# marbl/Mash

Hardware: AMD Instinct MI355X
Metric: pairwise Mash distances/sec (s=1000) (higher is better)
Workload: dtype u64; 1 GPU; mash triangle all-vs-all, 100000 clustered synthetic sketches, k=21 s=1000, 4999950000 pairs/step, per-table job (index build + discover + fill + merge each step), row-block sharded x1; parallelism=rowblock1, rccl_ranks=0

## Files before the change

mash_amd/csrc/compare_dense.hip:

```cpp
#ifdef MG_HIP_EMU
#include "hipemu.h"
#else
#include <hip/hip_runtime.h>
#define MG_DYN_SHARED(T, name)                                   \
    extern __shared__ __align__(16) unsigned char name##_raw[]; \
    T *name = reinterpret_cast<T *>(name##_raw)
#endif
#include <stdint.h>

#include <cstdlib>

#ifndef MG_HIP_EMU
#include <rocprim/device/device_radix_sort.hpp>
#include <rocprim/device/device_select.hpp>
#include <rocprim/iterator/counting_iterator.hpp>
#endif

#include "compare_internal.h"

namespace mg {

#ifndef MG_HIP_EMU
__global__ __launch_bounds__(256) void dn_neighbor_kernel(const uint64_t *hashes, uint64_t stride, const uint32_t *cnt, uint32_t n,
                                                          uint8_t *link)
// ... 79 lines not shown
    if (lane == 63u) s_w[wid] = incl;
    __syncthreads();
    uint32_t base = 0;
    for (uint32_t k = 0; k < wid; k++) base += s_w[k];
    off[t] = base + incl - c;
    if (t == DN_SUBLISTS - 1u) total[0] = base + incl;
    atomicMax(&total[1], want);
}

__global__ __launch_bounds__(256) void dn_sublists_copy_kernel(const unsigned long long *key, const uint32_t *val, const uint32_t *cnt,
                                                               const uint32_t *off, uint32_t cap_sub, unsigned long long *key_out,
                                                               uint32_t *val_out)
{
    const uint32_t sub = blockIdx.x;
    const uint32_t c = cnt[sub] < cap_sub ? cnt[sub] : cap_sub, o = off[sub];
    for (uint32_t k = threadIdx.x; k < c; k += 256u) {
        key_out[o + k] = key[(uint64_t)sub * cap_sub + k];
        val_out[o + k] = val[(uint64_t)sub * cap_sub + k];
    }
}

__global__ __launch_bounds__(256) void dn_universe_split_kernel(const unsigned long long *key_sorted, uint32_t m, uint32_t *ulist,
                                                                uint32_t *ustart, uint32_t *uend)
{
    const uint32_t i = blockIdx.x * 256u + threadIdx.x;
    if (i >= m) return;
    const unsigned long long k = key_sorted[i];
    const uint32_t g = (uint32_t)(k >> 32);
    ulist[i] = (uint32_t)k;
    if (i == 0 || (uint32_t)(key_sorted[i - 1] >> 32) != g) ustart[g] = i;
    if (i + 1u == m || (uint32_t)(key_sorted[i + 1] >> 32) != g) uend[g] = i + 1u;
}

size_t dense_universe_temp_bytes(uint32_t cap)
{
    size_t b = 0;
    rocprim::radix_sort_pairs(nullptr, b, (const unsigned long long *)nullptr, (unsigned long long *)nullptr, (const uint32_t *)nullptr,
                              (uint32_t *)nullptr, (size_t)cap, 0u, 64u, (hipStream_t) nullptr);
    return b;
}

uint32_t dense_sublists() { return DN_SUBLISTS; }

hipError_t dense_find_leaders(const uint32_t *sorted_rows, const uint32_t *gs_of, const uint32_t *gend, const uint32_t *grp_of,
                              const DenseGroup *groups, uint32_t E, unsigned long long *key, uint32_t *val, uint32_t cap_sub,
                              unsigned long long *key_out, uint32_t *val_out, uint32_t *cnt, uint32_t *off, uint32_t *total,
                              hipStream_t stream)
{
    if (E == 0) return hipSuccess;
    hipError_t e = hipMemsetAsync(cnt, 0, DN_SUBLISTS * 4, stream);
    if (e == hipSuccess) e = hipMemsetAsync(total, 0, 8, stream);
    if (e != hipSuccess) return e;
    hipLaunchKernelGGL(dn_leaders_kernel, dim3((E + 255u) / 256u), dim3(256), 0, stream, sorted_rows, gs_of, gend, grp_of, groups, E, key, val, cap_sub,
                       cnt);
    e = hipGetLastError();
    if (e != hipSuccess) return e;
    return dense_join_leaders(key, val, cap_sub, key_out, val_out, cnt, off, total, stream);
}

hipError_t dense_join_leaders(const unsigned long long *key, const uint32_t *val, uint32_t cap_sub, unsigned long long *key_out, uint32_t *val_out,
                              const uint32_t *cnt, uint32_t *off, uint32_t *total, hipStream_t stream)
{
    hipLaunchKernelGGL(dn_sublists_scan_kernel, dim3(1), dim3(DN_SUBLISTS), 0, stream, cnt, cap_sub, off, total);
    hipLaunchKernelGGL(dn_sublists_copy_kernel, dim3(DN_SUBLISTS), dim3(256), 0, stream, key, val, cnt, (const uint32_t *)off, cap_sub, key_out, val_out);
    return hipGetLastError();
}

hipError_t dense_sort_universes(const unsigned long long *key, const uint32_t *val, uint32_t m, void *temp, size_t temp_bytes,
                                unsigned long long *key_sorted, uint32_t *ulist, uint32_t *upos, uint32_t *ustart, uint32_t *uend,
                                uint32_t group_bits, hipStream_t stream)
{
    if (m == 0) return hipSuccess;
    hipError_t e = rocprim::radix_sort_pairs(temp, temp_bytes, key, key_sorted, val, upos, (size_t)m, 0u, 32u + group_bits, stream);
    if (e != hipSuccess) return e;
    hipLaunchKernelGGL(dn_universe_split_kernel, dim3((m + 255u) / 256u), dim3(256), 0, stream, (const unsigned long long *)key_sorted, m, ulist,
                       ustart, uend);
    return hipGetLastError();
}

#endif

constexpr uint32_t DN_CX_MASK = 0x7FFFu, DN_CX_FLAG = 0x8000u;

template <uint32_t DN_EK>
__global__ __launch_bounds__(256) void dn_encode_kernel(const uint32_t *off, const uint32_t *code_img, uint32_t *pos_img, uint32_t rs,
                                                        const uint32_t *grp_of, const DenseGroup *groups, const uint32_t *ulist,
                                                        const uint32_t *upos, unsigned long long *gdata, uint32_t wstride, uint16_t *ext,
                                                        uint32_t xs, uint32_t n, uint32_t ul_in_lds)
{
    MG_DYN_SHARED(uint32_t, lds);
    const uint32_t bid = blockIdx.x;
    const uint32_t row = (bid & ~63u) | ((bid & 7u) << 3) | ((bid >> 3) & 7u);
    const uint32_t tid = threadIdx.x, lane = tid & 63u, wid = tid >> 6;
    if (row >= n) return;
    const uint32_t g = grp_of[row];
    if (g == 0xFFFFFFFFu) return;
    const DenseGroup G = groups[g];
    const uint32_t W = G.W, u = G.u;
    uint32_t *mask32 = lds, *hist = lds + 2u * W, *gap8 = hist + W + 1u, *ovf = gap8 + 16u * W, *pl32 = ovf + W, *scr = pl32 + 8u * W;
    uint32_t *ull = lds + 28u * wstride + 9u;
    for (uint32_t i = tid; i < 28u * W + 1u; i += 256u) lds[i] = 0;
    const uint32_t *ulg = ulist + G.ustart, *up = upos + G.ustart;
    if (ul_in_lds)
        for (uint32_t i = tid; i < u; i += 256u) ull[i] = ulg[i];
    const uint32_t *ul = ul_in_lds ? ull : ulg;
    __syncthreads();
    const uint32_t cnt = off[row + 1] - off[row];
    uint16_t *xrow = ext + (uint64_t)(G.xrow0 + (row - G.g0)) * xs;
    uint32_t nx = 0;
    if constexpr (DN_EK == 1) {
        for (uint32_t base = 0; base < cnt; base += 256u) {
            const uint32_t p = base + tid;
            uint32_t idx = 0;
            bool extra = false;
            if (p < cnt) {
                const uint64_t img = (uint64_t)row * rs + p;
                const uint32_t gs = code_img[img] >> 1;
                uint32_t lo = 0, hi = u;
                while (lo < hi) {
                    const uint32_t mid = (lo + hi) >> 1;
                    if (ul[mid] < gs) lo = mid + 1; else hi = mid;
                }
                idx = lo;
                if (lo < u && ul[lo] == gs) {
                    atomicOr(&mask32[idx >> 5], 1u << (idx & 31u));
                    pos_img[img] = up[idx];
                } else {
                    extra = true;
                }
            }
            const uint64_t bal = __ballot(extra);
            const uint32_t before = (uint32_t)__popcll(bal & ((1ull << lane) - 1ull));
            if (lane == 0) scr[wid] = (uint32_t)__popcll(bal);
            __syncthreads();
            uint32_t woff = 0;
            for (uint32_t k = 0; k < wid; k++) woff += scr[k];
            const uint32_t total = scr[0] + scr[1] + scr[2] + scr[3];
            if (extra) {
                xrow[nx + woff + before] = (uint16_t)idx;
                atomicAdd(&hist[idx >> 6], 1u);
                atomicAdd(&gap8[idx >> 2], 1u << (8u * (idx & 3u)));
            }
            nx += total;
            __syncthreads();
        }
    } else {
        for (uint32_t base = 0; base < cnt; base += 256u * DN_EK) {
            const uint32_t p0 = base + tid * DN_EK;
            const uint32_t nv = p0 < cnt ? (cnt - p0 < DN_EK ? cnt - p0 : DN_EK) : 0u;
            uint32_t xidx[DN_EK];
            uint32_t nxt = 0;
            if (nv) {
                const uint64_t img0 = (uint64_t)row * rs + p0;
                const uint4 c0 = *reinterpret_cast<const uint4 *>(code_img + img0), c1 = *reinterpret_cast<const uint4 *>(code_img + img0 + 4u);
                const uint32_t code[DN_EK] = {c0.x, c0.y, c0.z, c0.w, c1.x, c1.y, c1.z, c1.w};
                uint4 *pp = reinterpret_cast<uint4 *>(pos_img + img0);
                const uint4 q0 = pp[0], q1 = pp[1];
                uint32_t pv[DN_EK] = {q0.x, q0.y, q0.z, q0.w, q1.x, q1.y, q1.z, q1.w};
                uint32_t pos = 0;
                {
                    const uint32_t gs0 = code[0] >> 1;
                    uint32_t lo = 0, hi = u;
                    while (lo < hi) {
                        const uint32_t mid = (lo + hi) >> 1;
                        if (ul[mid] < gs0) lo = mid + 1; else hi = mid;
                    }
                    pos = lo;
                }
    #pragma unroll
                for (uint32_t e = 0; e < DN_EK; e++) {
                    if (e < nv) {
                        const uint32_t gs = code[e] >> 1;
                        {
                            uint32_t lo = pos, hi = pos, step = 1;
                            while (hi < u && ul[hi] < gs) {
                                lo = hi + 1u;
                                hi += step;
                                step <<= 1;
                            }
                            hi = hi < u ? hi : u;
                            while (lo < hi) {
                                const uint32_t mid = (lo + hi) >> 1;
                                if (ul[mid] < gs) lo = mid + 1u; else hi = mid;
                            }
                            pos = lo;
                        }
                        if (pos < u && ul[pos] == gs) {
                            atomicOr(&mask32[pos >> 5], 1u << (pos & 31u));
                            pv[e] = up[pos];
                        } else {
    #pragma unroll
                            for (uint32_t j = 0; j < DN_EK; j++)
                                if (j == nxt) xidx[j] = pos;
                            nxt++;
                        }
                    }
                }
                pp[0] = make_uint4(pv[0], pv[1], pv[2], pv[3]);
                pp[1] = make_uint4(pv[4], pv[5], pv[6], pv[7]);
            }
            uint32_t incl = nxt;
    #pragma unroll
            for (uint32_t d = 1; d < 64u; d <<= 1) {
                const uint32_t y = __shfl_up(incl, d);
                if (lane >= d) incl += y;
            }
            if (lane == 63u) scr[wid] = incl;
            __syncthreads();
            uint32_t woff = 0;
            for (uint32_t k = 0; k < wid; k++) woff += scr[k];
            const uint32_t total = scr[0] + scr[1] + scr[2] + scr[3];
            const uint32_t at0 = nx + woff + incl - nxt;
    #pragma unroll
            for (uint32_t j = 0; j < DN_EK; j++) {
                if (j < nxt) {
                    const uint32_t idx = xidx[j];
                    xrow[at0 + j] = (uint16_t)idx;
                    atomicAdd(&hist[idx >> 6], 1u);
                    atomicAdd(&gap8[idx >> 2], 1u << (8u * (idx & 3u)));
                }
            }
            nx += total;
            __syncthreads();
        }
    }
    __syncthreads();
    const uint32_t jb = (row - G.g0) >> 7, bl = (row - G.g0) & 127u;
    const uint64_t bw = dense_block_words(W);
    unsigned long long *blk = gdata + G.data_off + (uint64_t)jb * bw;
    uint16_t *cxp = reinterpret_cast<uint16_t *>(blk + 128ull * W), *totp = cxp + (W + 1u) * 128u;
    unsigned long long *xpl = blk + dense_block_planes(W);
    for (uint32_t i = tid; i < 16u * W; i += 256u) {
        const uint32_t four = gap8[i], w = i >> 4, q = i & 15u;
        uint32_t bits[4] = {0u, 0u, 0u, 0u}, over = 0;
#pragma unroll
        for (uint32_t e = 0; e < 4u; e++) {
            const uint32_t c = (four >> (8u * e)) & 255u;
            over |= c >= 16u ? 1u : 0u;
#pragma unroll
            for (uint32_t j = 0; j < 4u; j++) bits[j] |= ((c >> j) & 1u) << ((4u * q + e) & 31u);
        }
        if (over || (q == 0 && hist[w] >= 256u)) ovf[w] = 1u;
#pragma unroll
        for (uint32_t j = 0; j < 4u; j++)
            if (bits[j]) atomicOr(&pl32[2u * (4u * w + j) + (q >> 3)], bits[j]);
    }
    __syncthreads();
    for (uint32_t i = tid; i < 4u * W; i += 256u) xpl[i * 128u + bl] = (unsigned long long)pl32[2u * i] | ((unsigned long long)pl32[2u * i + 1u] << 32);
    if (tid == 0) {
        uint32_t run = 0, all = 0;
        for (uint32_t w = 0; w <= W; w++) {
            cxp[w * 128u + bl] = (uint16_t)(run | ((w > 0 && ovf[w - 1u]) ? DN_CX_FLAG : 0u));
            totp[w * 128u + bl] = (uint16_t)all;
            if (w < W) {
                run += hist[w];
                all += hist[w] + (uint32_t)__popc(mask32[2u * w]) + (uint32_t)__popc(mask32[2u * w + 1u]);
            }
        }
    }
    for (uint32_t w = tid; w < W; w += 256u)
        blk[w * 128u + bl] = (unsigned long long)mask32[2u * w] | ((unsigned long long)mask32[2u * w + 1u] << 32);
}

hipError_t launch_dense_encode(const uint32_t *off, const uint32_t *code_img, uint32_t *pos_img, uint32_t rs, const uint32_t *grp_of,
                               const DenseGroup *groups, const uint32_t *ulist, const uint32_t *upos, unsigned long long *gdata,
                               uint16_t *ext, uint32_t xs, uint32_t n, uint32_t wmax, hipStream_t stream, int ul_mode)
{
    if (n == 0) return hipSuccess;
    const size_t fixed = ((size_t)28 * wmax + 9) * 4, with_ul = fixed + (size_t)wmax * 64 * 4;
    const bool ul_in_lds = ul_mode == 0 ? false : ul_mode == 1 ? with_ul <= 150 * 1024 : with_ul <= 40 * 1024;
    const size_t smem = ul_in_lds ? with_ul : fixed;
    auto go = [&](auto kern) -> hipError_t {
        hipError_t e = hipFuncSetAttribute(reinterpret_cast<const void *>(kern), hipFuncAttributeMaxDynamicSharedMemorySize, (int)smem);
        if (e != hipSuccess) return e;
        hipLaunchKernelGGL(kern, dim3((n + 63u) & ~63u), dim3(256), smem, stream, off, code_img, pos_img, rs, grp_of, groups, ulist, upos, gdata, wmax, ext, xs,
                           n, ul_in_lds ? 1u : 0u);
        return hipGetLastError();
    };
    return rs >= 4096u ? go(dn_encode_kernel<8>) : go(dn_encode_kernel<1>);
}



__device__ __forceinline__ uint32_t dn_count_add(uint32_t x, uint32_t acc)
{
#ifdef MG_HIP_EMU
    return (uint32_t)__popc(x) + acc;
#else
    uint32_t d;
    asm("v_bcnt_u32_b32 %0, %1, %2" : "=v"(d) : "v"(x), "v"(acc));
    return d;
#endif
}

__device__ __forceinline__ uint32_t dn_low_bits(uint32_t x, uint32_t y)
{
#ifdef MG_HIP_EMU
    return x & ((1u << y) - 1u);
#else
    return __builtin_amdgcn_ubfe(x, 0u, y);
#endif
}

template <uint32_t NP>
__device__ __forceinline__ uint32_t dn_descend(uint32_t base, uint32_t s, uint32_t u1, uint32_t A0, uint32_t B0, uint32_t A1, uint32_t B1,
                                               uint32_t A2, uint32_t B2, uint32_t A3, uint32_t B3)
{
    uint32_t pos = 0;
#pragma unroll
    for (uint32_t bit = 16u; bit != 0u; bit >>= 1) {
        const uint32_t y = pos + bit;
        uint32_t c = dn_count_add(dn_low_bits(B0, y), dn_count_add(dn_low_bits(A0, y), dn_count_add(dn_low_bits(u1, y), base)));
        if (NP >= 1u) c += 2u * dn_count_add(dn_low_bits(B1, y), (uint32_t)__popc(dn_low_bits(A1, y)));
        if (NP >= 3u)
            c += 4u * dn_count_add(dn_low_bits(B2, y), (uint32_t)__popc(dn_low_bits(A2, y))) +
                 8u * dn_count_add(dn_low_bits(B3, y), (uint32_t)__popc(dn_low_bits(A3, y)));
        pos = c < s ? y : pos;
    }
    return pos;
}

__device__ __forceinline__ uint32_t dn_resolve(unsigned long long un, unsigned long long mab, uint32_t fprev, uint32_t s, uint32_t w, bool lists,
                                               const unsigned long long *xpa, const unsigned long long *xpb, const uint16_t *xa,
                                               const uint16_t *xb, uint32_t ca0, uint32_t na, uint32_t cb0, uint32_t nb)
{
    if (__ballot(lists) == 0) {
        const unsigned long long a0 = xpa[512u * w], a1 = xpa[512u * w + 128u], a2 = xpa[512u * w + 256u], a3 = xpa[512u * w + 384u];
        const unsigned long long b0 = xpb[512u * w], b1 = xpb[512u * w + 128u], b2 = xpb[512u * w + 256u], b3 = xpb[512u * w + 384u];
        const bool p1 = __ballot((a1 | b1) != 0ull) != 0, p23 = __ballot((a2 | a3 | b2 | b3) != 0ull) != 0;
        const uint32_t ulo = (uint32_t)un, uhi = (uint32_t)(un >> 32);
        uint32_t c31 = dn_count_add((uint32_t)b0, dn_count_add((uint32_t)a0, dn_count_add(ulo & 0x7FFFFFFFu, fprev)));
        if (p1 || p23) c31 += 2u * dn_count_add((uint32_t)b1, (uint32_t)__popc((uint32_t)a1));
        if (p23)
            c31 += 4u * dn_count_add((uint32_t)b2, (uint32_t)__popc((uint32_t)a2)) + 8u * dn_count_add((uint32_t)b3, (uint32_t)__popc((uint32_t)a3));
        const bool upper = c31 < s;
        const uint32_t base = upper ? c31 + (ulo >> 31) : fprev;
        const uint32_t u1 = (upper ? uhi : ulo) << 1;
        const uint32_t A0 = upper ? (uint32_t)(a0 >> 32) : (uint32_t)a0, B0 = upper ? (uint32_t)(b0 >> 32) : (uint32_t)b0;
        uint32_t pos;
        if (!p1 && !p23) {
            pos = dn_descend<0>(base, s, u1, A0, B0, 0, 0, 0, 0, 0, 0);
        } else {
            const uint32_t A1 = upper ? (uint32_t)(a1 >> 32) : (uint32_t)a1, B1 = upper ? (uint32_t)(b1 >> 32) : (uint32_t)b1;
            if (!p23) {
                pos = dn_descend<1>(base, s, u1, A0, B0, A1, B1, 0, 0, 0, 0);
            } else {
                const uint32_t A2 = upper ? (uint32_t)(a2 >> 32) : (uint32_t)a2, B2 = upper ? (uint32_t)(b2 >> 32) : (uint32_t)b2;
                const uint32_t A3 = upper ? (uint32_t)(a3 >> 32) : (uint32_t)a3, B3 = upper ? (uint32_t)(b3 >> 32) : (uint32_t)b3;
                pos = dn_descend<3>(base, s, u1, A0, B0, A1, B1, A2, B2, A3, B3);
            }
        }
        const uint32_t mlo = (uint32_t)mab, mhi = (uint32_t)(mab >> 32);
        return upper ? dn_count_add(dn_low_bits(mhi, pos), (uint32_t)__popc(mlo)) : (uint32_t)__popc(dn_low_bits(mlo, pos));
    }
    uint32_t lo = 0, hi = 63;
    const uint32_t wbase = w << 6;
    while (lo < hi) {
        const uint32_t mid = (lo + hi) >> 1;
        uint32_t c = fprev + (uint32_t)__popcll(un & ((1ull << mid) - 1ull));
// ... 292 lines not shown
```

mash_amd/csrc/compare_internal.h:

```cpp
#pragma once
#ifdef MG_HIP_EMU
#include "hipemu.h"
#else
#include <hip/hip_runtime.h>
#endif
#include <stdint.h>

namespace mg {

struct MergedTile {
    uint32_t rows[32];
    uint32_t col0, col1;
};

struct CompareArgs {
    const uint64_t *row_hashes;
    const uint32_t *row_nhash;
    const uint64_t *col_hashes;
    const uint32_t *col_nhash;
    const uint32_t *row_pfx;
    const uint32_t *col_pfx;
    const MergedTile *mtiles;
    uint2 *out;
    uint64_t row_stride, col_stride;
    uint64_t row_pfx_stride, col_pfx_stride;
    uint64_t row_begin, row_end;
    uint64_t ncols;
    uint64_t out_base;
    uint32_t s;
    uint32_t rows_per_tile;
    uint32_t triangle;
    uint32_t unroll;
    uint32_t pfx_shr;
    uint32_t nbuckets;
    unsigned long long *dbg;
    const uint32_t *row_win;
    const uint32_t *col_win;
    uint32_t win, nwin;
    uint32_t win_lo, win_hi;
    uint32_t win_ecap;
    uint8_t *win_mask;
    uint32_t win_kmax;
    uint32_t xcd_remap;
    uint32_t stage_pack;
};

bool compare_merged_supported(uint32_t s);
uint32_t compare_merged_rows(uint32_t s);
hipError_t launch_compare_merged(const CompareArgs &a, uint32_t ntiles, hipStream_t stream);
uint32_t compare_window_rows(uint32_t s);
uint32_t compare_window_entries();
uint32_t compare_window_row_entries();
hipError_t launch_window_offsets(const uint32_t *pfx, uint64_t pfx_stride, const uint32_t *nhash, uint64_t n, uint32_t s,
                                 uint32_t nwin, uint32_t delta, uint32_t *out, hipStream_t stream);
hipError_t launch_table_max(const uint64_t *hashes, const uint32_t *nhash, uint64_t n, uint64_t stride,
                            unsigned long long *out_max, hipStream_t stream);
hipError_t launch_row_classes(const uint64_t *hashes, const uint32_t *nhash, uint64_t n, uint64_t stride,
                              uint8_t *out, unsigned long long *last_out, hipStream_t stream);
uint64_t compare_pfx_stride(uint64_t s);
hipError_t launch_make_prefix(const uint64_t *hashes, const uint32_t *nhash, uint64_t n, uint64_t s,
                              uint64_t pfx_stride, uint32_t shr, uint32_t *out, hipStream_t stream);
hipError_t launch_compare_generic(const CompareArgs &a, hipStream_t stream);

struct DenseGroup;
struct SparseArgs {
    const uint32_t *sorted_rows;
    const uint32_t *lo_img;
    const uint32_t *hi_img;
    uint32_t lo_shift;
    const uint32_t *off;
    const uint32_t *row_img;
    const uint32_t *col_img;
    const uint32_t *col_cnt_off;
    uint32_t rs_row, rs_col;
    uint32_t row_begin, row_end;
    uint32_t ncols;
    uint32_t triangle;
    uint32_t s;
    uint64_t out_base;
    uint2 *cand;
    uint64_t cand_cap;
    unsigned long long *counters;
    uint2 *out;
    uint2 *res;
    unsigned long long *seg_base;
    uint32_t *seg_cnt;
    uint32_t *chunk_inc;
    const uint32_t *rep;
    const uint32_t *cls_of;
    const uint32_t *cls_off;
    const uint32_t *cls_rows;
    const uint32_t *gend;
    const uint32_t *order;
    const uint32_t *inv;
    const uint32_t *dn_grp_of;
    const DenseGroup *dn_groups;
};
size_t sparse_dup_temp_bytes(uint32_t n);
hipError_t launch_sparse_dup_suspects(const unsigned long long *dig, const uint32_t *cnt, uint32_t n, void *temp, size_t temp_bytes,
                                      unsigned long long *dig_sorted, uint32_t *rows_sorted, uint32_t *flags, uint32_t *nflag,
                                      hipStream_t stream);
size_t sparse_order_temp_bytes(uint32_t n);
hipError_t launch_sparse_row_order(const uint32_t *off, const uint32_t *code_img, const uint32_t *gend, const uint32_t *rep, uint32_t n,
                                   uint32_t rs, void *temp, size_t temp_bytes, unsigned long long *key_a, unsigned long long *key_b,
                                   uint32_t *order, hipStream_t stream);
size_t sparse_order_slice_temp_bytes(uint32_t n);
hipError_t launch_sparse_order_slice(const uint32_t *order, uint32_t n, uint32_t rb, uint32_t re, void *temp, size_t temp_bytes,
                                     uint32_t *out, uint32_t *count_out, hipStream_t stream);
hipError_t launch_sparse_class_pairs(uint2 *out, const uint32_t *cls_rows, const uint32_t *cls_first, const uint32_t *off,
                                     const uint32_t *rep, uint32_t members, uint32_t row_begin, uint32_t row_end, uint64_t out_base,
                                     const uint32_t *inv, hipStream_t stream);
hipError_t launch_sparse_row_digest(const uint64_t *hashes, uint64_t stride, const uint32_t *cnt, uint32_t n,
                                    unsigned long long *digest, hipStream_t stream);
hipError_t launch_sparse_row_gate(const uint64_t *hashes, uint64_t stride, const uint32_t *cnt, uint32_t n, unsigned long long *digest,
                                  hipStream_t stream);
hipError_t launch_sparse_row_equal(const uint64_t *hashes, uint64_t stride, const uint32_t *cnt, const uint2 *pairs, uint32_t npairs,
                                   uint32_t *equal, hipStream_t stream);
hipError_t launch_sparse_row_counts(const uint32_t *nhash, uint32_t n, uint32_t cap, uint32_t *cnt, hipStream_t stream);
size_t sparse_offsets_temp_bytes(uint32_t n);
hipError_t launch_sparse_offsets(const uint32_t *cnt, const uint32_t *inv, uint32_t n, void *temp, uint32_t *off, hipStream_t stream);
size_t sparse_sort_temp_bytes(uint32_t E, uint32_t end_bit, uint32_t begin_bit);
uint32_t sparse_img_stride(uint32_t s);
hipError_t sparse_build_index(const uint64_t *hashes, uint64_t stride, const uint32_t *off, uint32_t n, uint32_t E,
                              uint32_t rs, uint32_t end_bit, void *temp, size_t temp_bytes, uint64_t *keys_a,
                              uint32_t *idx_a, uint64_t *keys_sorted, uint32_t *idx_sorted, uint32_t *head, uint32_t *gs_of,
                              uint32_t *sorted_rows, uint32_t *gend, uint32_t *code_img, uint32_t *pos_img, void *stat_scratch,
                              uint32_t begin_bit, void *tie_scratch, unsigned long long *incidences, uint32_t *max_group, uint32_t *groups,
                              uint32_t *bad, uint32_t *tie_overflow, hipStream_t stream, const uint32_t *rowmap = nullptr);
size_t sparse_stat_scratch_bytes();
uint32_t sparse_sort_begin_bit(uint32_t E, uint32_t end_bit, const char *forced_bits, bool all_bits);
size_t sparse_tie_scratch_bytes();
hipError_t launch_sparse_locate(const uint64_t *qhashes, uint64_t qstride, const uint32_t *qoff, uint32_t q_begin, uint32_t nq,
                                const uint64_t *keys_sorted, const uint32_t *gend, uint32_t E, uint32_t rs, uint32_t *qlo_img,
                                uint32_t *qhi_img, uint32_t *qcode_img, hipStream_t stream);
bool sparse_discover_supported(uint32_t ncols_max);
hipError_t launch_sparse_discover(const SparseArgs &a, bool count_only, hipStream_t stream);
hipError_t launch_sparse_merge(const SparseArgs &a, uint64_t expect, uint32_t cus, hipStream_t stream);
bool sparse_merge_rows_supported(uint32_t rs_row);
size_t sparse_scan_temp_bytes(uint32_t nrows);
hipError_t launch_sparse_merge_rows(const SparseArgs &a, uint64_t expect, uint32_t *chunks, void *temp, size_t temp_bytes,
                                    hipStream_t stream, bool *windowed_out = nullptr);
hipError_t launch_sparse_scatter(const SparseArgs &a, uint64_t expect, uint32_t cus, hipStream_t stream);
size_t sparse_gather_temp_bytes(uint32_t nrows);
hipError_t launch_sparse_gather_rows(const SparseArgs &a, uint32_t *cnt_by_row, uint32_t *row_base, void *temp, size_t temp_bytes, uint32_t row_add,
                                     uint2 *rc_out, uint2 *counts_out, hipStream_t stream);
size_t sparse_edges_temp_bytes(uint64_t K);
uint64_t sparse_edges_blocks(uint64_t K);
hipError_t launch_sparse_list_edges(const uint2 *rc, const uint2 *counts, uint64_t K, uint32_t *blk_cnt, uint32_t *blk_off, void *temp, size_t temp_bytes,
                                    uint4 *edges, unsigned long long *total, hipStream_t stream);
uint64_t sparse_fill_chunks(uint64_t pairs);
constexpr uint32_t kFillStop = 0x80000000u;
hipError_t launch_sparse_fill_chunks(uint2 *out, uint64_t pairs, uint32_t numer, uint32_t denom, uint32_t blocks, uint32_t naps, uint32_t *ctr,
                                     hipStream_t stream, uint32_t threads = 256);
hipError_t launch_sparse_fill_value(uint2 *out, uint64_t pairs, uint32_t numer, uint32_t denom, uint32_t blocks_per_cu, uint32_t cus,
                                    hipStream_t stream);
hipError_t launch_sparse_merge_pack(const SparseArgs &a, uint64_t expect, uint32_t *chunks, void *temp, size_t temp_bytes, bool *used,
                                    hipStream_t stream, uint32_t *pack_min_out = nullptr);
hipError_t launch_sparse_fill_short(uint2 *out, const uint32_t *short_rows, const uint32_t *short_rcnt, uint32_t nshort_rows,
                                    const uint32_t *short_cols, const uint32_t *short_ccnt, uint32_t nshort_cols,
                                    uint32_t row_begin, uint32_t ncols, uint32_t triangle, uint64_t out_base, uint32_t s,
                                    const uint32_t *inv, hipStream_t stream);

struct DenseGroup {
    uint32_t g0, g1;
    uint32_t ustart, u;
    uint32_t W;
    uint32_t xrow0;
    uint64_t data_off;
};
struct DenseTile { uint32_t group, row0, cblk; };
#ifdef __HIPCC__
__host__ __device__
#endif
static inline uint64_t dense_block_planes(uint32_t W) { return 128ull * W + 64ull * (W + 1u); }
#ifdef __HIPCC__
__host__ __device__
#endif
static inline uint64_t dense_block_words(uint32_t W) { return dense_block_planes(W) + 512ull * W; }
struct DenseList {
    const uint32_t *row_base = nullptr, *row_cnt = nullptr;
    uint2 *rc = nullptr, *counts = nullptr;
    uint32_t row_first = 0;
};
hipError_t launch_dense_neighbors(const uint64_t *hashes, uint64_t stride, const uint32_t *cnt, uint32_t n, uint8_t *link,
                                  hipStream_t stream);
size_t dense_universe_temp_bytes(uint32_t cap);
uint32_t dense_sublists();
hipError_t dense_find_leaders(const uint32_t *sorted_rows, const uint32_t *gs_of, const uint32_t *gend, const uint32_t *grp_of,
                              const DenseGroup *groups, uint32_t E, unsigned long long *key, uint32_t *val, uint32_t cap_sub,
                              unsigned long long *key_out, uint32_t *val_out, uint32_t *cnt, uint32_t *off, uint32_t *total,
                              hipStream_t stream);
hipError_t dense_join_leaders(const unsigned long long *key, const uint32_t *val, uint32_t cap_sub, unsigned long long *key_out, uint32_t *val_out,
                              const uint32_t *cnt, uint32_t *off, uint32_t *total, hipStream_t stream);
hipError_t dense_sort_universes(const unsigned long long *key, const uint32_t *val, uint32_t m, void *temp, size_t temp_bytes,
                                unsigned long long *key_sorted, uint32_t *ulist, uint32_t *upos, uint32_t *ustart, uint32_t *uend,
                                uint32_t group_bits, hipStream_t stream);
hipError_t launch_dense_encode(const uint32_t *off, const uint32_t *code_img, uint32_t *pos_img, uint32_t rs, const uint32_t *grp_of,
                               const DenseGroup *groups, const uint32_t *ulist, const uint32_t *upos, unsigned long long *gdata,
                               uint16_t *ext, uint32_t xs, uint32_t n, uint32_t wmax, hipStream_t stream, int ul_mode = -1);
size_t dense_pairs_lds(uint32_t W, uint32_t rows);
uint32_t dense_rows_per_tile(uint64_t wave_rows);
uint32_t dense_max_words();
hipError_t launch_dense_pairs(const DenseTile *tiles, uint32_t ntiles, uint32_t rows_per_tile, const DenseGroup *groups,
                              const unsigned long long *gdata, bool use_lists, const uint16_t *ext, uint32_t xs,
                              uint32_t s, uint32_t wmax, uint32_t row_begin, uint32_t row_end, uint64_t out_base, const uint32_t *inv, uint2 *out,
                              hipStream_t stream, const DenseList *list = nullptr);
size_t dense_cluster_temp_bytes(uint32_t n);
hipError_t dense_cluster_rows(const uint64_t *hashes, uint64_t stride, const uint32_t *cnt, uint32_t n, void *temp, size_t temp_bytes,
                              unsigned long long *key_a, unsigned long long *key_b, uint32_t *row_a, uint32_t *row_b, uint32_t *lab_a,
                              uint32_t *lab_b, uint32_t *inv, uint32_t *label_sorted, hipStream_t stream, uint32_t split = 0);
hipError_t launch_dense_gather_rows(const uint64_t *hashes, uint64_t stride, const uint32_t *inv, uint32_t n, uint64_t *out, hipStream_t stream);
hipError_t launch_dense_group_rows(const DenseGroup *groups, uint32_t ng, uint32_t n, uint32_t *grp_of, uint32_t *lead_rows, hipStream_t stream);

struct JoinSide {
    const uint2 *grp = nullptr;
    const uint32_t *ent = nullptr;
    const uint32_t *goff = nullptr;
    const uint32_t *gend = nullptr;
    const uint32_t *thr = nullptr;
};
struct JoinArgs {
    JoinSide rows, cols;
    const uint32_t *row_cnt_off, *col_cnt_off;
    const uint32_t *rep, *col_rep;
    const uint32_t *inv;
    uint2 *out;
    uint64_t out_base;
    uint64_t ntiles;
    uint32_t ncols;
    uint32_t row_begin, row_end;
    uint32_t bi0;
    uint32_t ncb;
    uint32_t triangle, s;
    uint32_t tiles_per_wg = 1;
};
size_t join_order_temp_bytes(uint32_t nrows);
hipError_t join_order_rows(const uint32_t *img, uint32_t rs, const uint32_t *cnt_off, const uint32_t *rep, const uint32_t *inv, const uint32_t *gend,
                           const uint32_t *sorted_rows, uint32_t nrows, void *temp, size_t temp_bytes, uint32_t *lab, unsigned long long *key_a,
                           unsigned long long *key_b, uint32_t *val_a, uint32_t *perm, uint32_t *src, uint32_t *map, hipStream_t stream, uint32_t split = 0);
uint32_t join_block_rows();
uint32_t join_levels();
size_t join_build_temp_bytes(uint64_t slots);
hipError_t join_build_lists(const uint32_t *img, uint32_t rs, const uint32_t *cnt_off, const uint32_t *rep, uint32_t nrows, uint32_t s, uint32_t E,
                            bool only_shared, void *temp, size_t temp_bytes, unsigned long long *key_a, unsigned long long *key_b, uint32_t *val_a,
                            uint32_t *val_b, uint2 *grp, uint32_t *goff, uint32_t *gend, uint32_t *thr, const uint32_t **ent_out, hipStream_t stream);
hipError_t launch_join_levels(const uint32_t *img, uint32_t rs, const uint32_t *cnt_off, const uint32_t *rep, uint32_t nrows, uint32_t s,
                              uint32_t *thr, hipStream_t stream);
hipError_t launch_join_shared(const uint32_t *lo_img, const uint32_t *hi_img, uint32_t lo_shift, uint32_t rs, const uint32_t *cnt_off,
                              uint32_t row_begin, uint32_t row_end, unsigned long long *sum, hipStream_t stream);
hipError_t launch_join_tiles(const JoinArgs &a, hipStream_t stream);

struct FilterArgs {
    const uint2 *counts;
    const uint32_t *min_numer;
    uint32_t *seg_count;
    unsigned long long *seg_off;
    uint4 *edges;
    uint64_t pairs;
    uint64_t first_row;
    uint64_t ncols;
    uint64_t win_lo, win_n;
    uint32_t s;
    uint32_t triangle;
};
uint64_t filter_segments(uint64_t pairs);
hipError_t launch_filter_count(const FilterArgs &a, unsigned long long *total, hipStream_t stream);
hipError_t launch_filter_write(const FilterArgs &a, hipStream_t stream);

}
```

mash_amd/csrc/compare_sparse.hip:

```cpp
#include <stdint.h>

#include <cstdlib>
#include <cstring>

#include "compare_internal.h"
#ifdef MG_HIP_EMU
#include <numeric>
#define SP_DYN_U32(name, align) MG_DYN_SHARED(uint32_t, name)
#else
#include <hip/hip_runtime.h>
#include <rocprim/device/device_radix_sort.hpp>
#include <rocprim/device/device_scan.hpp>
#include <rocprim/device/device_select.hpp>
#include <rocprim/iterator/counting_iterator.hpp>
#define SP_DYN_U32(name, align) extern __shared__ align uint32_t name[]
#endif
#include "copy_gate.h"

namespace mg {

#ifndef MG_HIP_EMU


__global__ __launch_bounds__(256) void sp_fill_entries_kernel(const uint64_t *hashes, uint64_t stride, const uint32_t *rowmap, const uint32_t *off,
// ... 517 lines not shown
        e = hipGetLastError();
        if (e != hipSuccess) return e;
    }
    hipLaunchKernelGGL(sp_heads_kernel, dim3(blocks), dim3(256), 0, stream, keys_sorted, idx_sorted, E, head, bad);
    e = hipGetLastError();
    if (e != hipSuccess) return e;
    e = rocprim::inclusive_scan(temp, temp_bytes, (const uint32_t *)head, gs_of, (size_t)E, sp_max_u32(), stream);
    if (e != hipSuccess) return e;
    {
        const uint64_t total = (uint64_t)n * rs;
        uint64_t fb = (total + 1023) / 1024;
        if (fb > 8192) fb = 8192;
        hipLaunchKernelGGL(sp_fill_u32_kernel, dim3((uint32_t)fb), dim3(256), 0, stream, code_img, total, 0xFFFFFFFFu);
        e = hipGetLastError();
        if (e != hipSuccess) return e;
    }
    e = hipMemsetAsync(stat_scratch, 0, sparse_stat_scratch_bytes(), stream);
    if (e != hipSuccess) return e;
    hipLaunchKernelGGL(sp_index_scatter_kernel, dim3(blocks), dim3(256), 0, stream, (const uint32_t *)idx_sorted, (const uint32_t *)gs_of, E, rs,
                       sorted_rows, gend, code_img, pos_img, static_cast<SpStatSlot *>(stat_scratch));
    e = hipGetLastError();
    if (e != hipSuccess) return e;
    hipLaunchKernelGGL(sp_stat_reduce_kernel, dim3(1), dim3(256), 0, stream, static_cast<const SpStatSlot *>(stat_scratch), incidences, max_group,
                       groups);
    return hipGetLastError();
}

#endif


__global__ __launch_bounds__(256) void sp_locate_kernel(const uint64_t *qhashes, uint64_t qstride, const uint32_t *qoff,
                                                        uint32_t q_begin, uint32_t nq, const uint64_t *keys_sorted,
                                                        const uint32_t *gend, uint32_t E, uint32_t rs, uint32_t *qlo_img,
                                                        uint32_t *qhi_img, uint32_t *qcode_img)
{
    const uint32_t q = blockIdx.x;
    if (q >= nq) return;
    const uint32_t cnt = qoff[q + 1] - qoff[q];
    const uint64_t *src = qhashes + (uint64_t)(q_begin + q) * qstride;
    for (uint32_t p = threadIdx.x; p < cnt; p += 256) {
        const uint64_t v = src[p];
        uint32_t lo = 0, hi = E;
        while (lo < hi) {
            const uint32_t mid = lo + ((hi - lo) >> 1);
            if (keys_sorted[mid] < v) lo = mid + 1; else hi = mid;
        }
        const bool found = lo < E && keys_sorted[lo] == v;
        const uint64_t at = (uint64_t)q * rs + p;
        qcode_img[at] = found ? (lo << 1) + 1u : (lo << 1);
        qlo_img[at] = lo;
        qhi_img[at] = found ? gend[lo] : lo;
    }
}


__device__ __forceinline__ uint32_t sp_class_span(const SparseArgs &a, uint32_t c, uint32_t row, uint32_t &first)
{
    const uint32_t k = a.cls_of[c];
    if (k == 0xFFFFFFFFu) { first = 0xFFFFFFFFu; return 1u; }
    const uint32_t lo = a.cls_off[k], hi = a.cls_off[k + 1];
    first = lo;
    if (!a.triangle) return hi - lo;
    uint32_t l = lo, h = hi;
    while (l < h) {
        const uint32_t mid = (l + h) >> 1;
        if (a.cls_rows[mid] < row) l = mid + 1; else h = mid;
    }
    return l - lo;
}

template <bool COUNT_ONLY, bool DEDUP>
__global__ __launch_bounds__(256) void sp_discover_kernel(SparseArgs a)
{
    SP_DYN_U32(bm, );
    __shared__ uint32_t s_w[4];
    __shared__ unsigned long long s_base;
    __shared__ unsigned long long s_inc[4];
    const uint32_t row = a.order ? a.order[blockIdx.x] : a.row_end - 1u - blockIdx.x;
    const uint32_t tid = threadIdx.x, lane = tid & 63u, wid = tid >> 6;
    const uint32_t ncols = a.triangle ? row : a.ncols;
    const uint32_t W = (ncols + 31u) >> 5;
    const uint32_t er = (DEDUP && a.triangle) ? a.rep[row] : row;
    const bool copy = DEDUP && a.triangle && er != row;
    const uint32_t cnt = a.off[er + 1] - a.off[er];
    if (cnt == 0 || ncols == 0) return;
    if (!copy) {
        int any = 0;
        for (uint32_t p = tid; p < cnt; p += 256u) {
            const uint64_t at = (uint64_t)er * a.rs_row + p;
            any |= (a.lo_img[at] >> a.lo_shift) != a.hi_img[at];
        }
        if (__syncthreads_or(any) == 0) return;
    }
    for (uint32_t w = tid; w < W; w += 256) bm[w] = 0;
    __syncthreads();
    unsigned long long inc = 0;
    constexpr uint32_t SHORT = 6;
    for (uint32_t base = wid * 64u; base < cnt; base += 256u) {
        const uint32_t p = base + lane;
        uint2 lh = make_uint2(0u, 0u);
        if (p < cnt) {
            const uint64_t at = (uint64_t)er * a.rs_row + p;
            lh = make_uint2(a.lo_img[at] >> a.lo_shift, a.hi_img[at]);
            if (copy) lh.y = a.gend[lh.x];
        }
        const uint32_t len = lh.y - lh.x;
        inc += len;
        if (len != 0 && len <= SHORT) {
            for (uint32_t t = 0; t < len; t++) {
                const uint32_t r = a.sorted_rows[lh.x + t];
                if (copy && r >= row) break;
                if (copy && r == er) continue;
                if (!((bm[r >> 5] >> (r & 31u)) & 1u)) atomicOr(&bm[r >> 5], 1u << (r & 31u));
            }
        }
        auto mark = [&](uint32_t r) {
            if (copy && (r >= row || r == er)) return;
            if (!((bm[r >> 5] >> (r & 31u)) & 1u)) atomicOr(&bm[r >> 5], 1u << (r & 31u));
        };
        uint64_t longm = __ballot(len > SHORT);
        while (longm != 0) {
            uint32_t lo4[4], hi4[4], r4[4];
#pragma unroll
            for (int k = 0; k < 4; k++) {
                lo4[k] = hi4[k] = 0;
                if (longm != 0) {
                    const int l = __builtin_ctzll(longm);
                    longm &= longm - 1;
                    lo4[k] = (uint32_t)__builtin_amdgcn_readlane((int)lh.x, l);
                    hi4[k] = (uint32_t)__builtin_amdgcn_readlane((int)lh.y, l);
                }
                r4[k] = lo4[k] + lane < hi4[k] ? a.sorted_rows[lo4[k] + lane] : 0xFFFFFFFFu;
            }
#pragma unroll
            for (int k = 0; k < 4; k++) {
                if (r4[k] != 0xFFFFFFFFu) mark(r4[k]);
                for (uint32_t q = lo4[k] + 64u + lane; q < hi4[k]; q += 64u) mark(a.sorted_rows[q]);
            }
        }
    }
    __syncthreads();
    const uint32_t per = (W + 255u) / 256u;
    const uint32_t w0 = tid * per, w1 = w0 + per < W ? w0 + per : W;
    uint32_t mine = 0;
    for (uint32_t w = w0; w < w1; w++) {
        if (!DEDUP) {
            mine += (uint32_t)__popc(bm[w]);
        } else {
            uint32_t bits = bm[w];
            while (bits != 0) {
                const uint32_t c = (w << 5) + (uint32_t)__builtin_ctz(bits);
                bits &= bits - 1;
                uint32_t first;
                mine += sp_class_span(a, c, row, first);
            }
        }
    }
    uint32_t incl = mine;
#pragma unroll
    for (int d = 1; d < 64; d <<= 1) {
        const uint32_t t = __shfl_up(incl, d);
        if (lane >= (uint32_t)d) incl += t;
    }
    for (int d = 32; d > 0; d >>= 1) inc += __shfl_xor(inc, d);
    if (lane == 63) s_w[wid] = incl;
    if (lane == 0) s_inc[wid] = inc;
    __syncthreads();
    uint32_t woff = 0;
    for (uint32_t w = 0; w < wid; w++) woff += s_w[w];
// ... 885 lines not shown
```

mash_amd/csrc/host_compare.cpp:

```cpp
#include "cut_internal.h"
#include "index_build.h"
#ifdef IX_PHASE_CLOCKS
namespace mg { void index_dump_clocks(); }
#endif
#include "sort_bits.h"
#include "topk_internal.h"
#include "knn_internal.h"
#include <type_traits>


int table_max(mg_ctx *ctx, const mg_table *t, uint64_t *out)
{
    if (!t->have_max) {
        unsigned long long *d = nullptr;
        HIP_TRY(ctx, hipMalloc(&d, 8));
        hipError_t e = hipMemsetAsync(d, 0, 8, ctx->stream);
        if (e == hipSuccess) e = mg::launch_table_max(t->hashes, t->nhash, t->n, t->s, d, ctx->stream);
        unsigned long long h = 0;
        if (e == hipSuccess) e = hipMemcpyAsync(&h, d, 8, hipMemcpyDeviceToHost, ctx->stream);
        if (e == hipSuccess) e = hipStreamSynchronize(ctx->stream);
        hipFree(d);
        if (e != hipSuccess) return fail(ctx, MG_ERR_HIP, std::string("table max: ") + hipGetErrorString(e));
        t->maxval = h;
        t->have_max = true;
// ... 507 lines not shown
        }
    }
    aside_wgs = wgs; aside_naps = naps; aside_threads = threads;
    ctx->aside_all_copies = [this](uint32_t c) { aside_other_constant(c); };
    uint64_t late_from = 300000000ull;
    if (const char *e = ctx_opt(ctx, "MASHGPU_FILL_ASIDE_AT_SORT")) late_from = strtoull(e, nullptr, 10);
    if (cols->n * std::min<uint64_t>(cols->s, s) >= late_from) {
        ctx->aside_at_sort = [this]() { (void)aside_start(); };
        return MG_OK;
    }
    return aside_start();
}

int SparseJobRun::aside_start()
{
    ctx->aside_at_sort = nullptr;
    if (prefilled) return MG_OK;
    HIP_TRY(ctx, hipMemsetAsync(ctx->aux_ctr, 0, 128, ctx->stream));
    HIP_TRY(ctx, hipEventRecord(ctx->aux_go, ctx->stream));
    HIP_TRY(ctx, hipStreamWaitEvent(ctx->aux, ctx->aux_go, 0));
    const bool copies = triangle && aside_copies != 0;
    return aside_launch(copies ? aside_copies : 0u, copies ? aside_copies : s, ctx->aux_ctr);
}

int SparseJobRun::aside_launch(uint32_t numer, uint32_t denom, uint32_t *ctr)
{
    prof_begin(ctx, ctx->prof_fill_aside, ctx->aux);
    HIP_TRY(ctx, mg::launch_sparse_fill_chunks(reinterpret_cast<uint2 *>(out_dev), pairs, numer, denom, aside_wgs, aside_naps, ctr, ctx->aux, aside_threads));
    prof_end(ctx, ctx->prof_fill_aside, ctx->aux);
    HIP_TRY(ctx, hipEventRecord(ctx->aux_done, ctx->aux));
    aside_numer = numer; aside_denom = denom; aside_ctr = ctr;
    prefilled = true;
    return MG_OK;
}

void SparseJobRun::aside_other_constant(uint32_t c)
{
    aside_copies = c;
    if (!prefilled || !triangle) return;
    if (hipMemsetAsync(aside_ctr, 0x80, 4, ctx->stream) != hipSuccess || aside_launch(c, c, ctx->aux_ctr + 16) != MG_OK) (void)hipGetLastError();
}

int SparseJobRun::end_prefill(bool finish)
{
    ctx->aside_all_copies = nullptr;
    ctx->aside_at_sort = nullptr;
    if (!prefilled) return MG_OK;
    prefilled = false;
    hipError_t e;
    if (finish) e = mg::launch_sparse_fill_chunks(reinterpret_cast<uint2 *>(out_dev), pairs, aside_numer, aside_denom, (uint32_t)ctx->cu_count * 16u, 0u, aside_ctr, ctx->stream);
    else e = hipMemsetAsync(aside_ctr, 0x80, 4, ctx->stream);
    const hipError_t e2 = hipStreamWaitEvent(ctx->stream, ctx->aux_done, 0);
    if (e != hipSuccess || e2 != hipSuccess) return fail(ctx, MG_ERR_HIP, std::string("compare (fill beside the build): ") + hipGetErrorString(e != hipSuccess ? e : e2));
    return MG_OK;
}

int SparseJobRun::row_side()
{
    a.sorted_rows = ix->sorted_rows;
    a.col_img = ix->code_img;
    a.col_cnt_off = ix->off;
    a.rs_col = ix->rs;
    a.ncols = (uint32_t)cols->n;
    a.triangle = triangle ? 1u : 0u;
    a.s = s;
    a.out = reinterpret_cast<uint2 *>(out_dev);
    a.counters = ix->counters;
    a.rep = ix->rep;
    a.cls_of = ix->cls_of;
    a.cls_off = ix->cls_off;
    a.cls_rows = ix->cls_rows;
    a.gend = ix->gend;
    a.inv = ix->inv;
    a.dn_grp_of = (job && triangle && !ix->dgroups_host.empty()) ? ix->grp_of : nullptr;
    a.dn_groups = a.dn_grp_of ? ix->dgroups : nullptr;
    a.res = nullptr;
    a.seg_base = nullptr;
    a.seg_cnt = nullptr;
    a.chunk_inc = nullptr;
    if (triangle) {
        a.lo_img = ix->code_img;
        a.hi_img = ix->pos_img;
        a.lo_shift = 1;
        a.off = ix->off;
        a.row_img = ix->code_img;
        a.rs_row = ix->rs;
        a.row_begin = (uint32_t)row_begin;
        a.row_end = (uint32_t)row_end;
        a.out_base = row_begin ? row_begin * (row_begin - 1) / 2 : 0;
        const auto &sr = ix->short_rows_host;
        const size_t k0 = std::lower_bound(sr.begin(), sr.end(), (uint32_t)row_begin) - sr.begin();
        const size_t k1 = std::lower_bound(sr.begin(), sr.end(), (uint32_t)row_end) - sr.begin();
        nshort_rows = (uint32_t)(k1 - k0);
        short_rows_dev = ix->short_rows ? ix->short_rows + k0 : nullptr;
        short_rcnt_dev = ix->short_cnt ? ix->short_cnt + k0 : nullptr;
    } else {
        rc = table_classes(ctx, rows);
        if (rc != MG_OK) return rc;
        std::vector<uint32_t> qoff(nrows + 1);
        uint64_t Eq = 0;
        for (uint64_t q = 0; q < nrows; q++) {
            qoff[q] = (uint32_t)Eq;
            const uint64_t c = std::min<uint64_t>(std::min<uint64_t>(rows->nh[row_begin + q], rows->s), s);
            Eq += c;
            if (Eq >= (1ull << 31)) return leave();
            if (c < s) { qshort_h.push_back((uint32_t)q); qshort_cnt_h.push_back((uint32_t)c); }
            if (c && rows->last[row_begin + q] == MG_HASH_PAD) return leave();
        }
        qoff[nrows] = (uint32_t)Eq;
        const uint32_t rsq = ix->rs;
        if (nrows * rsq >= (1ull << 32)) return leave();
        if (q_off.alloc(nrows + 1) != hipSuccess || q_img.alloc(nrows * rsq) != hipSuccess || q_lo.alloc(nrows * rsq) != hipSuccess ||
            q_hi.alloc(nrows * rsq) != hipSuccess || q_short.alloc(std::max<size_t>(qshort_h.size(), 1)) != hipSuccess ||
            q_short_cnt.alloc(std::max<size_t>(qshort_h.size(), 1)) != hipSuccess) {
            (void)hipGetLastError();
            return leave();
        }
        HIP_TRY(ctx, hipMemcpyAsync(q_off, qoff.data(), (nrows + 1) * 4, hipMemcpyHostToDevice, ctx->stream));
        if (!qshort_h.empty()) {
            HIP_TRY(ctx, hipMemcpyAsync(q_short, qshort_h.data(), qshort_h.size() * 4, hipMemcpyHostToDevice, ctx->stream));
            HIP_TRY(ctx, hipMemcpyAsync(q_short_cnt, qshort_cnt_h.data(), qshort_h.size() * 4, hipMemcpyHostToDevice, ctx->stream));
        }
        HIP_TRY(ctx, hipStreamSynchronize(ctx->stream));
        HIP_TRY(ctx, mg::launch_sparse_locate(rows->hashes, rows->s, q_off, (uint32_t)row_begin, (uint32_t)nrows, ix->keys_sorted, ix->gend,
                                              ix->E, rsq, q_lo, q_hi, q_img, ctx->stream));
        a.lo_img = q_lo;
        a.hi_img = q_hi;
        a.lo_shift = 0;
        a.off = q_off;
        a.row_img = q_img;
        a.rs_row = rsq;
        a.row_begin = 0;
        a.row_end = (uint32_t)nrows;
        a.out_base = 0;
        nshort_rows = (uint32_t)qshort_h.size();
        short_rows_dev = q_short;
        short_rcnt_dev = q_short_cnt;
    }
    return MG_OK;
}

int SparseJobRun::find_plan()
{
    if (triangle)
        for (auto &pl : ix->plans)
            if (pl.rows == (const void *)rows && pl.rb == row_begin && pl.re == row_end && pl.triangle == triangle) plan = &pl;
    fresh.order = nullptr;
    fresh.dtiles = nullptr;
    first = plan == nullptr;
    if (first) {
        fresh.rows = rows; fresh.rb = row_begin; fresh.re = row_end; fresh.triangle = triangle;
        fresh.cand = 0; fresh.shared = 0; fresh.use = true; fresh.use_list = true; fresh.join = false; fresh.order = nullptr;
        fresh.dtiles = nullptr; fresh.ndtiles = 0; fresh.dtile_rows = 32; fresh.dense_pairs = 0;
        if (triangle && !ix->dgroups_host.empty()) {
            uint64_t wave_rows = 0;
            for (const mg::DenseGroup &G : ix->dgroups_host) {
                const uint64_t m = G.g1 - G.g0;
                wave_rows += m * ((m + 127) / 128);
            }
            const uint32_t R = mg::dense_rows_per_tile(wave_rows);
            fresh.dtile_rows = R;
            std::vector<mg::DenseTile> tiles;
            for (uint32_t g = 0; g < ix->dgroups_host.size(); g++) {
                const mg::DenseGroup &G = ix->dgroups_host[g];
                if (G.g1 <= row_begin || G.g0 >= row_end) continue;
                for (uint32_t row0 = G.g0; row0 < G.g1; row0 += R) {
                    const uint64_t a_lo = std::max<uint64_t>(std::max<uint64_t>(row0, row_begin), (uint64_t)G.g0 + 1), a_hi = std::min<uint64_t>(std::min<uint64_t>(row0 + R, G.g1), row_end);
                    if (a_lo >= a_hi) continue;
                    for (uint64_t ra = a_lo; ra < a_hi; ra++) fresh.dense_pairs += ra - G.g0;
                    const uint32_t cb_last = (uint32_t)((a_hi - 2 - G.g0) >> 7);
                    for (uint32_t cb = 0; cb <= cb_last; cb++) tiles.push_back({g, row0, cb});
                }
            }
            if (!tiles.empty()) {
                void *q = nullptr;
                if (ctx_malloc(ctx, &q, tiles.size() * sizeof(mg::DenseTile)) != hipSuccess) { (void)hipGetLastError(); return fail(ctx, MG_ERR_NOMEM, "compare: no device memory for the dense tiles"); }
                hipError_t e = hipMemcpyAsync(q, tiles.data(), tiles.size() * sizeof(mg::DenseTile), hipMemcpyHostToDevice, ctx->stream);
                if (e == hipSuccess) e = hipStreamSynchronize(ctx->stream);
                if (e != hipSuccess) { ctx_free(ctx, q); return fail(ctx, MG_ERR_HIP, std::string("compare (dense tiles): ") + hipGetErrorString(e)); }
                fresh.dtiles = static_cast<mg::DenseTile *>(q);
                fresh.ndtiles = (uint32_t)tiles.size();
            }
        }
        if (triangle && ix->order) {
            if (row_begin == 0 && row_end == cols->n) {
                fresh.order = nullptr;
            } else {
                void *q = nullptr, *tmp = nullptr, *cnt = nullptr;
                const size_t tb = mg::sparse_order_slice_temp_bytes((uint32_t)cols->n);
                if (ctx_malloc(ctx, &q, nrows * 4) == hipSuccess && ctx_malloc(ctx, &tmp, std::max<size_t>(tb, 16)) == hipSuccess &&
                    ctx_malloc(ctx, &cnt, 8) == hipSuccess &&
                    mg::launch_sparse_order_slice(ix->order, (uint32_t)cols->n, (uint32_t)row_begin, (uint32_t)row_end, tmp, tb,
                                                  static_cast<uint32_t *>(q), static_cast<uint32_t *>(cnt), ctx->stream) == hipSuccess) {
                    fresh.order = static_cast<uint32_t *>(q);
                    q = nullptr;
                } else {
                    (void)hipGetLastError();
                }
                ctx_free(ctx, q);
                ctx_free(ctx, tmp);
                ctx_free(ctx, cnt);
            }
        }
        plan = &fresh;
    }
    a.order = triangle && ix->order ? (plan->order ? plan->order : (row_begin == 0 && row_end == cols->n ? ix->order : nullptr)) : nullptr;
    return MG_OK;
}

int SparseJobRun::ensure_lists(uint64_t want_cand)
{
    if (want_cand > ix->cand_cap) {
        for (void **q : {(void **)&ix->cand, (void **)&ix->res})
            if (*q) { ctx_free(ctx, *q); *q = nullptr; }
        ix->cand_cap = 0;
        const uint64_t cap = want_cand + want_cand / 8 + 1024;
        void *c1 = nullptr, *c2 = nullptr;
        if (ctx_malloc(ctx, &c1, cap * sizeof(uint2)) != hipSuccess || ctx_malloc(ctx, &c2, cap * sizeof(uint2)) != hipSuccess) {
            (void)hipGetLastError();
            ctx_free(ctx, c1);
            return fail(ctx, MG_ERR_NOMEM, "compare: no device memory for the candidate list");
        }
        ix->cand = static_cast<uint2 *>(c1);
        ix->res = static_cast<uint2 *>(c2);
        ix->cand_cap = cap;
    }
    if (nrows > ix->seg_rows) {
        for (void **q : {(void **)&ix->seg_base, (void **)&ix->seg_cnt, (void **)&ix->chunks, (void **)&ix->chunk_inc, &ix->scan_temp})
            if (*q) { ctx_free(ctx, *q); *q = nullptr; }
        ix->seg_rows = 0;
        const uint64_t cap = nrows + nrows / 8 + 256;
        ix->scan_temp_bytes = mg::sparse_scan_temp_bytes((uint32_t)cap);
        void *p1 = nullptr, *p2 = nullptr, *p3 = nullptr, *p4 = nullptr, *p5 = nullptr;
        if (ctx_malloc(ctx, &p1, cap * 8) != hipSuccess || ctx_malloc(ctx, &p2, cap * 4) != hipSuccess ||
            ctx_malloc(ctx, &p3, cap * 4) != hipSuccess || ctx_malloc(ctx, &p4, cap * 4) != hipSuccess ||
            ctx_malloc(ctx, &p5, std::max<size_t>(ix->scan_temp_bytes, 16)) != hipSuccess) {
            (void)hipGetLastError();
            for (void *q : {p1, p2, p3, p4, p5}) ctx_free(ctx, q);
            return fail(ctx, MG_ERR_NOMEM, "compare: no device memory for the merge work list");
        }
        ix->seg_base = static_cast<unsigned long long *>(p1);
        ix->seg_cnt = static_cast<uint32_t *>(p2);
        ix->chunks = static_cast<uint32_t *>(p3);
        ix->chunk_inc = static_cast<uint32_t *>(p4);
        ix->scan_temp = p5;
        ix->seg_rows = cap;
    }
    return MG_OK;
}

int SparseJobRun::discover()
{
    if (!first && !force && !(job ? plan->use_list : plan->use)) return leave();
    want = first ? std::max<uint64_t>(ix->cand_cap, std::min<uint64_t>(pairs, std::min<uint64_t>(std::max<uint64_t>((uint64_t)ix->E / 2, 1u << 16), 1ull << 27)))
                          : plan->cand;
    nothing_to_find = triangle && ix->one_class != 0;
    for (int attempt = 0; !nothing_to_find; attempt++) {
        rc = ensure_lists(want);
        if (rc != MG_OK) return rc;
        a.cand = ix->cand;
        a.res = ix->res;
        a.cand_cap = ix->cand_cap;
        a.seg_base = ix->seg_base;
        a.seg_cnt = ix->seg_cnt;
        a.chunk_inc = ix->chunk_inc;
        HIP_TRY(ctx, hipMemsetAsync(ix->counters, 0, 4 * 8, ctx->stream));
        HIP_TRY(ctx, hipMemsetAsync(ix->seg_cnt, 0, nrows * 4, ctx->stream));
        prof_begin(ctx, ctx->prof_discover);
        if (attempt == 0) clk_begin(CK_DISCOVER);
        hipError_t e = mg::launch_sparse_discover(a, false, ctx->stream);
        if (attempt == 0) clk_end(CK_DISCOVER);
        prof_end(ctx, ctx->prof_discover);
        if (e != hipSuccess) return fail(ctx, MG_ERR_HIP, std::string("compare (discover): ") + hipGetErrorString(e));
        if (!first) break;
        HIP_TRY(ctx, hipMemcpyAsync(h, ix->counters, 24, hipMemcpyDeviceToHost, ctx->stream));
        HIP_TRY(ctx, hipStreamSynchronize(ctx->stream));
        if (h[2] == 0) break;
        if (attempt >= 1) return fail(ctx, MG_ERR_INVALID, "compare: the table changed while it was compared");
        want = h[0];
    }
    return MG_OK;
}

int SparseJobRun::choose_engine()
{
    if (first) {
        fresh.cand = h[0];
        fresh.shared = h[1];
        const double np = (double)pairs;
        const SparseCosts &K = costs();
        const double t_sparse = np * 8.0 / K.fill_bytes_s + (double)fresh.shared * K.discover_per_shared + (double)nrows * s * K.discover_per_entry +
                                (double)fresh.cand * K.merge_per_candidate + K.launches + (triangle ? (double)ix->cls_pairs * 8.0 / K.class_bytes_s : 0.0) +
                                (double)fresh.dense_pairs * K.dense_per_pair;
        const double dense_rate = np < 3.0e8 ? K.tiles_rate_small : np < 2.0e9 ? K.tiles_rate_mid : K.tiles_rate_large;
        const double t_dense = np / dense_rate + (double)fresh.shared * K.tiles_per_shared;
        fresh.use = t_sparse < t_dense;
        fresh.use_list = t_sparse - np * 8.0 / K.fill_bytes_s - (triangle ? (double)ix->cls_pairs * 8.0 / K.class_bytes_s : 0.0) < t_dense;
        if (ctx_opt(ctx, "MASHGPU_SPARSE_DBG"))
            fprintf(stderr, "compare sparse: rows [%llu, %llu) %s: %llu pairs, %llu candidates, %llu shared hashes; model sparse %.3f ms, tiles %.3f ms\n",
                    (unsigned long long)row_begin, (unsigned long long)row_end, triangle ? "triangle" : "rect", (unsigned long long)pairs,
                    (unsigned long long)fresh.cand, (unsigned long long)fresh.shared, t_sparse * 1e3, t_dense * 1e3);
        keep_plan();
    }
    if (!force && !(job ? plan->use_list : plan->use)) return leave();
    return MG_OK;
}

int SparseJobRun::keep_plan()
{
    if (!triangle || fresh_kept) return MG_OK;
    if (ix->plans.size() >= 64) {
        if (ix->plans.front().order) ctx_free(ctx, ix->plans.front().order);
        if (ix->plans.front().dtiles) ctx_free(ctx, ix->plans.front().dtiles);
        ix->plans.erase(ix->plans.begin());
    }
    ix->plans.push_back(fresh);
    fresh_kept = true;
    plan = &ix->plans.back();
    return MG_OK;
}

struct JoinListBufs {
    mg_ctx *ctx;
    void *bufs[6] = {nullptr, nullptr, nullptr, nullptr, nullptr, nullptr};
    mg::JoinSide side;
    explicit JoinListBufs(mg_ctx *c) : ctx(c) {}
    ~JoinListBufs() { for (void *q : bufs) if (q) ctx_free(ctx, q); }
    void release_to(void **out) { for (int i = 0; i < 6; i++) { out[i] = bufs[i]; bufs[i] = nullptr; } }
};

static int join_make_lists(mg_ctx *ctx, const uint32_t *img, uint32_t rs, const uint32_t *cnt_off, const uint32_t *rep, uint32_t nrows, uint32_t s,
                           uint32_t E, bool only_shared, JoinListBufs &L)
{
    const uint64_t slots = (uint64_t)nrows * s;
    const uint32_t nblocks = (nrows + mg::join_block_rows() - 1u) / mg::join_block_rows();
    const size_t tb = mg::join_build_temp_bytes(slots);
    DevBuf<unsigned long long> key_a(ctx), key_b(ctx);
    DevBuf<unsigned char> temp(ctx);
    bool ok = key_a.alloc(slots) == hipSuccess && key_b.alloc(slots) == hipSuccess && temp.alloc(std::max<size_t>(tb, 16)) == hipSuccess;
// ... 1342 lines not shown
```

mash_amd/csrc/host_index.cpp:

```cpp
#include "host_internal.h"
#include "index_build.h"
#ifdef IX_PHASE_CLOCKS
namespace mg { void index_dump_clocks(); }
#endif
#include "sort_bits.h"

namespace {

const uint64_t kTilesLongestRun = 6144;
static const uint64_t kSplitMinRun = 128;

uint64_t longest_label_run(const uint32_t *lab_sorted, uint64_t n)
{
    if (!lab_sorted || n == 0) return 0;
    uint64_t run = 1, longest = 1;
    for (uint64_t a = 1; a < n; a++) {
        run = lab_sorted[a] == lab_sorted[a - 1] ? run + 1 : 1;
        longest = std::max(longest, run);
    }
    return longest;
}

struct Carve {
    unsigned char *base = nullptr;
// ... 57 lines not shown
    bool cluster_q = false, links_q = false;

    const char *ix_mode = nullptr;
    bool ix_verify = false, ix_tiles = true;
    std::vector<uint32_t> cnt_true, cnt_perm;
    uint32_t max_cnt = 0;
    uint64_t maxv = 0, E_all = 0;
    double dens[65] = {0};
    double dens0 = 0;
    std::vector<uint32_t> rep;
    const uint64_t *H = nullptr;
    const uint32_t *rowmap = nullptr;
    uint64_t label_run = 0;
    mg::IxPlan early_plan;
    DevBuf<unsigned char> d_lb;
    bool lb_made = false;
    DevBuf<unsigned char> d_tcnt;
    bool cnt_made = false;
    bool cnt_stale = false;

    std::vector<uint32_t> cls_of, cls_off, cls_rows, cls_first;

    uint32_t E = 0, end_bit = 0, sort_begin_bit = 0;
    std::vector<mg::DenseGroup> cand_groups;
    std::vector<uint32_t> grp_of_h;
    DevBuf<mg::DenseGroup> d_groups;
    DevBuf<uint32_t> d_grp_of, d_lead_rows;
    LeaderLists lead;
    bool lead_ready = false, cand_prepared = false;
    mg::IxPlan plan;
    size_t temp_bytes = 0;
    DevBuf<unsigned char> temp;
    DevBuf<uint32_t> gs_of;
    DevBuf<unsigned long long> key64_a, key64_b;
    struct Stat { unsigned long long shared; uint32_t max_group, groups, bad, tie_overflow; uint32_t ixf[4]; } h_stat = {0, 0, 0, 0, 0, {0, 0, 0, 0}};
    DevBuf<Stat> d_stat;
    DevBuf<unsigned char> d_slots;
    bool want_order = true;
    std::vector<uint32_t> short_cnt;

    bool built = false;
    uint64_t dn_xrows = 0, dn_words = 0;

    SparseIndexBuild(mg_ctx *c, const mg_table *tab, uint32_t sketch_size, bool clustered_variant, mg_table::Sparse *index, uint32_t split_row)
        : ctx(c), t(tab), s(sketch_size), clustered(clustered_variant), split(split_row), sp(index), n(tab->n), dc_cls(c), d_link(c), dc_last(c), d_dig(c), d_dig_sorted(c),
          k_a(c), k_b(c), d_cnt(c), d_rows_sorted(c), d_flags(c), d_nflag(c), r_a(c), r_b(c), l_a(c), l_b(c), d_inv(c), d_lab(c), d_tmp_dup(c), d_tmp_cl(c), d_lb(c), d_tcnt(c),
          d_groups(c), d_grp_of(c), d_lead_rows(c), lead(c), temp(c), gs_of(c), key64_a(c), key64_b(c), d_stat(c), d_slots(c)
    {}

    int unusable(const char *why) { sp->usable = false; sp->why = why; stop = true; return MG_OK; }


    bool counts_with_offsets()
    {
        const char *o = ctx_opt(ctx, "MASHGPU_IX_COUNTS");
        if ((o && strcmp(o, "tiles") == 0) || !mg::index_offsets_counts_fits(early_plan.g)) return false;
        if (d_tcnt.alloc(early_plan.cnt_bytes) != hipSuccess || d_stat.alloc(1) != hipSuccess ||
            hipMemsetAsync(d_stat, 0, sizeof(Stat), ctx->stream) != hipSuccess) {
            (void)hipGetLastError();
            d_tcnt.free();
            return false;
        }
        return cnt_made = true;
    }

    hipError_t counts_to_device()
    {
            if (!cnt_stale) return hipSuccess;
            cnt_stale = false;
            return hipMemcpyAsync(d_cnt, cnt_true.data(), n * 4, hipMemcpyHostToDevice, ctx->stream);
    }

    template <class T> bool take(T **p, size_t count)
    {
        void *q = nullptr;
        if (ctx_malloc(ctx, &q, std::max<size_t>(count, 1) * sizeof(T)) != hipSuccess) return false;
        *p = static_cast<T *>(q);
        return true;
    }

    void drop()
    {
            for (void **q : {(void **)&sp->off, (void **)&sp->keys_sorted, (void **)&sp->gend, (void **)&sp->sorted_rows, (void **)&sp->code_img,
                             (void **)&sp->pos_img, (void **)&sp->short_rows, (void **)&sp->short_cnt, (void **)&sp->counters, (void **)&sp->order,
                             (void **)&sp->rep, (void **)&sp->cls_of, (void **)&sp->cls_off, (void **)&sp->cls_rows, (void **)&sp->cls_first})
                if (*q) { ctx_free(ctx, *q); *q = nullptr; }
    }

    int no_memory() { (void)hipGetLastError(); drop(); return unusable("no device memory for the index"); }
    int lost(hipError_t e) { drop(); return fail(ctx, MG_ERR_HIP, std::string("compare (index build): ") + hipGetErrorString(e)); }

    void drop_dense()
    {
        for (void **q : {(void **)&sp->dgroups, (void **)&sp->grp_of, (void **)&sp->gdata, (void **)&sp->ext, (void **)&sp->ulist, (void **)&sp->upos})
            if (*q) { ctx_free(ctx, *q); *q = nullptr; }
        sp->dgroups_host.clear();
    }

    struct TileScratch {
        DevBuf<unsigned char> start, big, pk, tc;
        explicit TileScratch(mg_ctx *c) : start(c), big(c), pk(c), tc(c) {}
    };

    hipError_t tiles(const TileScratch &w, int stages)
    {
        const mg::IxLeaders lv = lead.view(d_lead_rows);
        return mg::index_build_mapped(plan, H, rowmap, sp->off, d_lb, d_tcnt, w.start, w.big, w.pk, w.tc, sp->keys_sorted, sp->sorted_rows, sp->gend, gs_of, sp->code_img,
                               sp->pos_img, d_slots, &d_stat.p->shared, &d_stat.p->max_group, &d_stat.p->groups, d_stat.p->ixf, lead_ready ? &lv : nullptr,
                               ctx->stream, stages);
    }
    hipError_t sort_buckets(const TileScratch &w)
    {
        hipError_t e = tiles(w, 2);
        if (e == hipSuccess && lead_ready) e = lead.join(ctx->stream);
        return e != hipSuccess ? e : hipMemcpyAsync(&h_stat, d_stat, sizeof(Stat), hipMemcpyDeviceToHost, ctx->stream);
    }
    hipError_t row_order()
    {
        return mg::launch_sparse_row_order(sp->off, sp->code_img, sp->gend, sp->rep, (uint32_t)n, sp->rs, temp, temp_bytes, key64_a, key64_b, sp->order, ctx->stream);
    }

    int scan_rows();
    int copy_rows();
    int order_rows();
    int find_copies();
    int lay_out();
    void prepare_candidates();
    hipError_t tile_passes();
    int build_by_tiles();
    int build_by_sort();
    int check_build();
    bool search_leaders();
    bool sort_universes(std::vector<uint32_t> &us, std::vector<uint32_t> &ue);
    bool choose_groups(const std::vector<uint32_t> &us, const std::vector<uint32_t> &ue);
    int encode_groups();
    int dense_groups();
    int run();
};

int SparseIndexBuild::scan_rows()
{
    need_classes = t->cls.size() != n;
    dedup = !ctx_opt(ctx, "MASHGPU_SPARSE_NO_DEDUP");
    want_dense = true;
    if (const char *v = ctx_opt(ctx, "MASHGPU_COMPARE_DENSE")) want_dense = atoi(v) != 0;
    try_cluster = clustered && n >= 16;
    try_links = !try_cluster && want_dense && n >= 8 && s <= 16384;
    tb_dup = mg::sparse_dup_temp_bytes((uint32_t)n);
    tb_cl = mg::dense_cluster_temp_bytes((uint32_t)n);
    if (d_cnt.alloc(n) != hipSuccess || (need_classes && (dc_cls.alloc(n) != hipSuccess || dc_last.alloc(n) != hipSuccess)) ||
        (dedup && (d_dig.alloc(n) != hipSuccess || d_dig_sorted.alloc(n) != hipSuccess || d_rows_sorted.alloc(n) != hipSuccess ||
                   d_flags.alloc(n) != hipSuccess || d_nflag.alloc(1) != hipSuccess || d_tmp_dup.alloc(std::max<size_t>(tb_dup, 16)) != hipSuccess))) {
        (void)hipGetLastError();
        return unusable("no device memory for the index");
    }
    {
        hipError_t e = hipSuccess;
        if (need_classes) {
            hc_cls.resize(n);
            hc_last.resize(n);
            hc_nh.resize(n);
            e = mg::launch_row_classes(t->hashes, t->nhash, n, t->s, dc_cls, dc_last, ctx->stream);
        }
        if (e == hipSuccess) e = mg::launch_sparse_row_counts(t->nhash, (uint32_t)n, (uint32_t)std::min<uint64_t>(t->s, s), d_cnt, ctx->stream);
        if (e == hipSuccess && dedup) {
            e = mg::launch_sparse_row_gate(t->hashes, t->s, d_cnt, (uint32_t)n, d_dig, ctx->stream);
            if (e == hipSuccess)
                e = mg::launch_sparse_dup_suspects(d_dig, d_cnt, (uint32_t)n, d_tmp_dup, tb_dup, d_dig_sorted, d_rows_sorted, d_flags, d_nflag, ctx->stream);
        }
        if (e == hipSuccess && try_cluster) {
            if (k_a.alloc(4 * n) == hipSuccess && k_b.alloc(4 * n) == hipSuccess && r_a.alloc(4 * n) == hipSuccess && r_b.alloc(4 * n) == hipSuccess &&
                l_a.alloc(n) == hipSuccess && l_b.alloc(n) == hipSuccess && d_inv.alloc(n) == hipSuccess && d_lab.alloc(n) == hipSuccess &&
                d_tmp_cl.alloc(std::max<size_t>(tb_cl, 16)) == hipSuccess) {
                e = mg::dense_cluster_rows(t->hashes, t->s, d_cnt, (uint32_t)n, d_tmp_cl, tb_cl, k_a, k_b, r_a, r_b, l_a, l_b, d_inv, d_lab, ctx->stream, split);
                cluster_q = true;
            } else {
                (void)hipGetLastError();
            }
        }
        if (e == hipSuccess && try_links) {
            if (d_link.alloc(n) == hipSuccess) {
                link.resize(n);
                e = mg::launch_dense_neighbors(t->hashes, t->s, d_cnt, (uint32_t)n, d_link, ctx->stream);
                links_q = true;
            } else {
                (void)hipGetLastError();
            }
        }
        unsigned long long *p_last = nullptr;
        uint32_t *p_nh = nullptr, *p_inv = nullptr, *p_lab = nullptr, *p_nflag = nullptr;
        uint8_t *p_cls = nullptr, *p_link = nullptr;
        auto carve = [&](unsigned char *block) {
            Carve c{block};
            p_last = c.take<unsigned long long>(n); p_nh = c.take<uint32_t>(n); p_inv = c.take<uint32_t>(n); p_lab = c.take<uint32_t>(n);
            p_nflag = c.take<uint32_t>(2); p_cls = c.take<uint8_t>(n); p_link = c.take<uint8_t>(n);
            return c.at + 64;
        };
        unsigned char *pin = static_cast<unsigned char *>(ctx_pinned(ctx, carve(nullptr)));
        if (pin) {
            carve(pin);
        } else {
            p_nflag = &nflag;
            if (cluster_q) { inv_v.resize(n); lab_v.resize(n); p_inv = inv_v.data(); p_lab = lab_v.data(); }
            p_nh = hc_nh.data(); p_cls = hc_cls.data(); p_last = reinterpret_cast<unsigned long long *>(hc_last.data()); p_link = link.data();
        }
        if (e == hipSuccess && need_classes) {
            e = hipMemcpyAsync(p_nh, t->nhash, n * 4, hipMemcpyDeviceToHost, ctx->stream);
            if (e == hipSuccess) e = hipMemcpyAsync(p_cls, dc_cls, n, hipMemcpyDeviceToHost, ctx->stream);
            if (e == hipSuccess) e = hipMemcpyAsync(p_last, dc_last, n * 8, hipMemcpyDeviceToHost, ctx->stream);
        }
        if (e == hipSuccess && dedup) e = hipMemcpyAsync(p_nflag, d_nflag, 4, hipMemcpyDeviceToHost, ctx->stream);
        if (e == hipSuccess && cluster_q) {
            e = hipMemcpyAsync(p_inv, d_inv, n * 4, hipMemcpyDeviceToHost, ctx->stream);
            if (e == hipSuccess) e = hipMemcpyAsync(p_lab, d_lab, n * 4, hipMemcpyDeviceToHost, ctx->stream);
        }
        if (e == hipSuccess && links_q) e = hipMemcpyAsync(p_link, d_link, n, hipMemcpyDeviceToHost, ctx->stream);
        const hipError_t es = hipStreamSynchronize(ctx->stream);
        if (e == hipSuccess) e = es;
        if (e == hipSuccess && pin) {
// ... 132 lines not shown
            HIP_TRY(ctx, hipMemcpyAsync(rows_sorted.data(), d_rows_sorted, n * 4, hipMemcpyDeviceToHost, ctx->stream));
            HIP_TRY(ctx, hipMemcpyAsync(flags.data(), d_flags, n * 4, hipMemcpyDeviceToHost, ctx->stream));
            HIP_TRY(ctx, hipStreamSynchronize(ctx->stream));
            std::vector<uint2> pairs;
            pairs.reserve(nflag);
            for (uint64_t k = 1, g0 = 0; k < n; k++) {
                if (flags[k]) pairs.push_back(make_uint2(rows_sorted[k], rows_sorted[g0]));
                else g0 = k;
            }
            DevBuf<uint2> d_pairs(ctx);
            DevBuf<uint32_t> d_eq(ctx);
            if (d_pairs.alloc(pairs.size()) != hipSuccess || d_eq.alloc(pairs.size()) != hipSuccess) { (void)hipGetLastError(); return unusable("no device memory for the index"); }
            std::vector<uint32_t> eq(pairs.size());
            HIP_TRY(ctx, hipMemcpyAsync(d_pairs, pairs.data(), pairs.size() * sizeof(uint2), hipMemcpyHostToDevice, ctx->stream));
            HIP_TRY(ctx, mg::launch_sparse_row_equal(H, t->s, d_cnt, d_pairs, (uint32_t)pairs.size(), d_eq, ctx->stream));
            HIP_TRY(ctx, hipMemcpyAsync(eq.data(), d_eq, pairs.size() * 4, hipMemcpyDeviceToHost, ctx->stream));
            HIP_TRY(ctx, hipStreamSynchronize(ctx->stream));
            for (size_t k = 0; k < pairs.size(); k++)
                if (eq[k]) {
                    if (rep.empty()) { rep.resize(n); for (uint64_t i = 0; i < n; i++) rep[i] = (uint32_t)i; }
                    rep[pairs[k].x] = pairs[k].y;
                    sp->copies++;
                }
        }
    }
    if (sp->copies) {
        cls_of.assign(n, 0xFFFFFFFFu);
        std::vector<uint32_t> size(n, 0);
        for (uint64_t i = 0; i < n; i++) size[rep[i]]++;
        uint32_t ncls = 0, tot = 0;
        for (uint64_t i = 0; i < n; i++)
            if (size[i] >= 2) { cls_of[i] = ncls++; cls_off.push_back(tot); tot += size[i]; }
        cls_off.push_back(tot);
        cls_rows.resize(tot);
        std::vector<uint32_t> fillp(cls_off.begin(), cls_off.end() - 1);
        for (uint64_t i = 0; i < n; i++) {
            const uint32_t k = cls_of[rep[i]];
            if (k != 0xFFFFFFFFu) cls_rows[fillp[k]++] = (uint32_t)i;
        }
        cls_first.resize(tot);
        for (uint32_t k = 0; k < ncls; k++) {
            const uint64_t m = cls_off[k + 1] - cls_off[k];
            sp->cls_pairs += m * (m - 1) / 2;
            for (uint32_t u = cls_off[k]; u < cls_off[k + 1]; u++) cls_first[u] = cls_off[k];
        }
        sp->cls_members = tot;
        if (ncls == 1 && tot == n && cnt_true[0] > 0) sp->one_class = (uint32_t)cnt_true[0];
        if (sp->one_class && ctx->aside_all_copies) ctx->aside_all_copies(sp->one_class);
    }
    return MG_OK;
}

int SparseIndexBuild::lay_out()
{
    uint64_t E64 = 0;
    sp->off_host.resize(n + 1);
    for (uint64_t i = 0; i < n; i++) {
        sp->off_host[i] = (uint32_t)E64;
        const uint64_t c = cnt_true[i];
        if (rep.empty() || rep[i] == i) E64 += c;
        if (E64 >= (1ull << 31)) return unusable("2^31 entries or more");
        if (c < s) sp->short_rows_host.push_back((uint32_t)i);
        if (c == 0) sp->has_empty = true;
    }
    sp->off_host[n] = (uint32_t)E64;
    if (E64 == 0) return unusable("no hashes");
    E = (uint32_t)E64;
    sp->E = E;
    end_bit = (uint32_t)(64 - __builtin_clzll(maxv | 1ull));
    sort_begin_bit = mg::sparse_sort_begin_bit(E, end_bit, ctx_opt(ctx, "MASHGPU_SPARSE_SORT_BITS"), ctx_opt(ctx, "MASHGPU_SPARSE_SORT_ALL_BITS") != nullptr);
    if (sort_begin_bit > 0 && !ctx_opt(ctx, "MASHGPU_SPARSE_SORT_BITS")) sort_begin_bit = mg::sort_begin_bit_from_density(dens, end_bit, sort_begin_bit);
    const bool tiles_hopeless = ix_tiles && !ix_verify && lab_sorted && !ctx_opt(ctx, "MASHGPU_SPARSE_INDEX") &&
                                label_run > kTilesLongestRun;
    if (ix_tiles && !tiles_hopeless) plan = mg::index_plan((uint32_t)n, E, s, sp->rs, t->s, maxv, dens0, ix_verify);
    else if (tiles_hopeless) plan.why = "a clade of more rows than a bucket's sort takes";
    if (lb_made && !(plan.ok && memcmp(&plan.g, &early_plan.g, sizeof plan.g) == 0)) lb_made = cnt_made = false;
    temp_bytes = std::max(std::max(mg::sparse_order_temp_bytes((uint32_t)n), mg::sparse_order_slice_temp_bytes((uint32_t)n)),
                          mg::sparse_offsets_temp_bytes((uint32_t)n));
    want_order = !ctx_opt(ctx, "MASHGPU_SPARSE_NO_ORDER");
    bool ok = temp.alloc(std::max<size_t>(temp_bytes, 16)) == hipSuccess && gs_of.alloc(E) == hipSuccess && (d_stat.p || d_stat.alloc(1) == hipSuccess) &&
              d_slots.alloc(std::max(mg::sparse_stat_scratch_bytes(), mg::index_stat_scratch_bytes())) == hipSuccess &&
              (!want_order || (key64_a.alloc(n) == hipSuccess && key64_b.alloc(n) == hipSuccess));
    ok = ok && take(&sp->off, n + 1) && take(&sp->keys_sorted, E) && take(&sp->gend, E) && take(&sp->sorted_rows, E) &&
         take(&sp->code_img, (size_t)n * sp->rs + 64) && take(&sp->pos_img, (size_t)n * sp->rs) && take(&sp->counters, 4) &&
         (!want_order || take(&sp->order, n));
    const size_t nshort = sp->short_rows_host.size();
    short_cnt.assign(nshort, 0);
    for (size_t k = 0; k < nshort; k++) short_cnt[k] = cnt_true[sp->short_rows_host[k]];
    if (ok && nshort) ok = take(&sp->short_rows, nshort) && take(&sp->short_cnt, nshort);
    if (ok && sp->copies)
        ok = take(&sp->rep, n) && take(&sp->cls_of, n) && take(&sp->cls_off, cls_off.size()) && take(&sp->cls_rows, cls_rows.size()) &&
             take(&sp->cls_first, cls_first.size());
    if (!ok) return no_memory();
    hipError_t e = hipSuccess;
    auto upload = [&](uint32_t *dst, const std::vector<uint32_t> &v) {
        if (e == hipSuccess && !v.empty()) e = hipMemcpyAsync(dst, v.data(), v.size() * 4, hipMemcpyHostToDevice, ctx->stream);
    };
    if (sp->copies) { upload(sp->rep, rep); upload(sp->cls_of, cls_of); upload(sp->cls_off, cls_off); upload(sp->cls_rows, cls_rows); upload(sp->cls_first, cls_first); }
    if (!rep.empty()) upload(sp->off, sp->off_host);
    else if (e == hipSuccess) e = mg::launch_sparse_offsets(d_cnt, cnt_stale ? sp->inv : nullptr, (uint32_t)n, temp, sp->off, ctx->stream);
    upload(sp->short_rows, sp->short_rows_host); upload(sp->short_cnt, short_cnt);
    return e == hipSuccess ? MG_OK : lost(e);
}

void SparseIndexBuild::prepare_candidates()
{
    if (cand_prepared) return;
    cand_prepared = true;
    if (link.empty() || sp->copies != 0) return;
    for (uint64_t i = 1; i < n;) {
        if (!link[i]) { i++; continue; }
        uint64_t j = i;
        while (j < n && link[j]) j++;
        if (j - (i - 1) >= 8) {
            mg::DenseGroup g{};
            g.g0 = (uint32_t)(i - 1); g.g1 = (uint32_t)j;
            cand_groups.push_back(g);
        }
        i = j + 1;
    }
    if (cand_groups.empty()) return;
    const uint32_t ng = (uint32_t)cand_groups.size();
    grp_of_h.assign(n, 0xFFFFFFFFu);
    for (uint32_t g = 0; g < ng; g++)
        for (uint32_t r = cand_groups[g].g0; r < cand_groups[g].g1; r++) grp_of_h[r] = g;
    uint32_t room = std::max<uint32_t>(E / 4u / lead.lists + 64u, 256u);
    if (const char *ev = ctx_opt(ctx, "MASHGPU_DENSE_LEAD_CAP")) room = std::max<uint32_t>((uint32_t)atoi(ev), 1u);
    if (d_groups.alloc(ng) == hipSuccess && d_grp_of.alloc(n) == hipSuccess && d_lead_rows.alloc(4 * n) == hipSuccess && lead.alloc(room) == hipSuccess &&
        hipMemcpyAsync(d_groups, cand_groups.data(), ng * sizeof(mg::DenseGroup), hipMemcpyHostToDevice, ctx->stream) == hipSuccess &&
        mg::launch_dense_group_rows(d_groups, ng, (uint32_t)n, d_grp_of, d_lead_rows, ctx->stream) == hipSuccess && lead.reset(ctx->stream) == hipSuccess) {
        lead_ready = true;
    } else {
        (void)hipGetLastError();
        cand_groups.clear();
    }
}

hipError_t SparseIndexBuild::tile_passes()
{
    TileScratch w(ctx);
    if (!((lb_made || d_lb.alloc(plan.lb_bytes) == hipSuccess) && (cnt_made || d_tcnt.alloc(plan.cnt_bytes) == hipSuccess) && w.start.alloc(plan.start_bytes) == hipSuccess &&
          w.big.alloc(plan.big_bytes) == hipSuccess && w.pk.alloc(plan.pk_bytes) == hipSuccess && w.tc.alloc(plan.tc_bytes) == hipSuccess)) {
        (void)hipGetLastError();
        return hipSuccess;
    }
    hipError_t e = cnt_made ? hipSuccess : hipMemsetAsync(d_stat, 0, sizeof(Stat), ctx->stream);
    if (e == hipSuccess) e = tiles(w, cnt_made ? 1 | 8 | 16 : lb_made ? 1 | 8 : 1);
    DevBuf<uint32_t> d_swapped(ctx);
    if (e == hipSuccess && ctx_opt(ctx, "MASHGPU_IX_DEBUG_SWAP") && d_swapped.alloc(1) == hipSuccess) {
        e = hipMemsetAsync(d_swapped, 0, 4, ctx->stream);
        if (e == hipSuccess) e = mg::index_debug_swap(plan, w.pk, w.start, d_swapped, ctx->stream);
    }
    if (e == hipSuccess) prepare_candidates();
    if (e == hipSuccess && ctx->aside_at_sort) ctx->aside_at_sort();
    if (e == hipSuccess) e = sort_buckets(w);
    hipEvent_t ev_stats = nullptr;
    if (e == hipSuccess) e = hipEventCreateWithFlags(&ev_stats, hipEventDisableTiming);
    if (e == hipSuccess) e = hipEventRecord(ev_stats, ctx->stream);
    if (e == hipSuccess) e = tiles(w, 4);
    if (e == hipSuccess && want_order) e = row_order();
    const hipError_t ew = e == hipSuccess ? hipEventSynchronize(ev_stats) : hipStreamSynchronize(ctx->stream);
    if (e == hipSuccess) e = ew;
    if (ev_stats) (void)hipEventDestroy(ev_stats);
    built = e == hipSuccess && !h_stat.ixf[mg::IXF_DEGENERATE];
    if (built && lead_ready && lead.overflowed() && h_stat.ixf[mg::IXF_NBIG] == 0) {
        e = hipStreamSynchronize(ctx->stream);
        const uint32_t want_cap = lead.tot[1];
// ... 96 lines not shown
        return fail(ctx, MG_ERR_INVALID, "index verify: tiles / sort -- " + msg + geom);
    }
    return MG_OK;
}

int SparseIndexBuild::check_build()
{
    if (h_stat.bad) { drop(); return unusable("sort order inside a value not by row"); }
    sp->G = h_stat.groups;
    sp->shared = h_stat.shared;
    sp->max_group = h_stat.max_group;
    sp->build_ms = std::chrono::duration<double, std::milli>(std::chrono::steady_clock::now() - t_begin).count();
    sp->usable = true;
    return MG_OK;
}

bool SparseIndexBuild::search_leaders()
{
    for (int attempt = 0;; attempt++) {
        hipError_t e = mg::dense_find_leaders(sp->sorted_rows, gs_of, sp->gend, d_grp_of, d_groups, E, lead.key, lead.val, lead.cap, lead.keyj, lead.valj,
                                              lead.cnt_sub, lead.off_sub, lead.nlead, ctx->stream);
        if (e == hipSuccess) e = hipMemcpyAsync(lead.tot, lead.nlead, 8, hipMemcpyDeviceToHost, ctx->stream);
        if (e == hipSuccess) e = hipStreamSynchronize(ctx->stream);
        if (e != hipSuccess) return false;
        if (!lead.overflowed() || attempt >= 1) return true;
        if (lead.alloc(lead.tot[1]) != hipSuccess) return false;
    }
}

bool SparseIndexBuild::sort_universes(std::vector<uint32_t> &us, std::vector<uint32_t> &ue)
{
    const uint32_t ng = (uint32_t)cand_groups.size(), nlead = lead.tot[0];
    uint32_t gbits = 1;
    while ((1u << gbits) < ng) gbits++;
    const size_t tb = mg::dense_universe_temp_bytes(nlead);
    DevBuf<uint32_t> d_us(ctx), d_ue(ctx);
    DevBuf<unsigned long long> d_key2(ctx);
    DevBuf<unsigned char> d_utmp(ctx);
    bool ok = d_us.alloc(ng) == hipSuccess && d_ue.alloc(ng) == hipSuccess && d_key2.alloc(nlead) == hipSuccess && d_utmp.alloc(std::max<size_t>(tb, 16)) == hipSuccess;
    if (!ok || !take(&sp->ulist, nlead) || !take(&sp->upos, nlead)) return false;
    hipError_t e = hipMemsetAsync(d_us, 0, ng * 4, ctx->stream);
    if (e == hipSuccess) e = hipMemsetAsync(d_ue, 0, ng * 4, ctx->stream);
    if (e == hipSuccess) e = mg::dense_sort_universes(lead.keyj, lead.valj, nlead, d_utmp, tb, d_key2, sp->ulist, sp->upos, d_us, d_ue, gbits, ctx->stream);
    if (e == hipSuccess) e = hipMemcpyAsync(us.data(), d_us, ng * 4, hipMemcpyDeviceToHost, ctx->stream);
    if (e == hipSuccess) e = hipMemcpyAsync(ue.data(), d_ue, ng * 4, hipMemcpyDeviceToHost, ctx->stream);
    if (e == hipSuccess) e = hipStreamSynchronize(ctx->stream);
    return e == hipSuccess;
}

bool SparseIndexBuild::choose_groups(const std::vector<uint32_t> &us, const std::vector<uint32_t> &ue)
{
    const uint32_t kMaxWords = mg::dense_max_words();
    std::fill(grp_of_h.begin(), grp_of_h.end(), 0xFFFFFFFFu);
    for (uint32_t g = 0; g < (uint32_t)cand_groups.size(); g++) {
        mg::DenseGroup G = cand_groups[g];
        G.u = ue[g] > us[g] ? ue[g] - us[g] : 0u;
        G.ustart = us[g];
        G.W = (G.u >> 6) + 1u;
        if (G.u < 32u || G.W > kMaxWords) continue;
        G.xrow0 = (uint32_t)dn_xrows;
        G.data_off = dn_words;
        const uint64_t m = G.g1 - G.g0;
        dn_xrows += m;
        dn_words += ((m + 127) / 128) * mg::dense_block_words(G.W);
        sp->dn_wmax = std::max(sp->dn_wmax, G.W);
        for (uint32_t r = G.g0; r < G.g1; r++) grp_of_h[r] = (uint32_t)sp->dgroups_host.size();
        sp->dgroups_host.push_back(G);
    }
    return !sp->dgroups_host.empty();
}

int SparseIndexBuild::encode_groups()
{
    sp->dn_xs = ((s + 7u) & ~7u) + 8u;
    if (!take(&sp->dgroups, sp->dgroups_host.size()) || !take(&sp->grp_of, n) || !take(&sp->gdata, dn_words) || !take(&sp->ext, dn_xrows * sp->dn_xs)) {
        (void)hipGetLastError();
        sp->dgroups_host.clear();
        return MG_OK;
    }
    hipError_t e = hipMemcpyAsync(sp->dgroups, sp->dgroups_host.data(), sp->dgroups_host.size() * sizeof(mg::DenseGroup), hipMemcpyHostToDevice, ctx->stream);
    if (e == hipSuccess) e = hipMemcpyAsync(sp->grp_of, grp_of_h.data(), n * 4, hipMemcpyHostToDevice, ctx->stream);
    if (e == hipSuccess)
        e = mg::launch_dense_encode(sp->off, sp->code_img, sp->pos_img, sp->rs, sp->grp_of, sp->dgroups, sp->ulist, sp->upos, sp->gdata, sp->ext, sp->dn_xs,
                                    (uint32_t)n, sp->dn_wmax, ctx->stream, ctx_opt(ctx, "MASHGPU_DENSE_UL_LDS") ? atoi(ctx_opt(ctx, "MASHGPU_DENSE_UL_LDS")) : -1);
    sp->grp_of_host.swap(grp_of_h);
    if (e != hipSuccess) {
        drop();
        drop_dense();
        sp->usable = false;
        return fail(ctx, MG_ERR_HIP, std::string("compare (index build, dense groups): ") + hipGetErrorString(e));
    }
    sp->dn_lists = ctx_opt(ctx, "MASHGPU_DENSE_LISTS") != nullptr;
    return MG_OK;
}

int SparseIndexBuild::dense_groups()
{
    if (!cand_groups.empty()) {
        auto t_dense = std::chrono::steady_clock::now();
        if (built && lead_ready && lead.overflowed() && ctx_opt(ctx, "MASHGPU_SPARSE_DBG"))
            fprintf(stderr, "compare dense: a list of leaders asked for %u entries, room for %u: no dense groups for this table\n", lead.tot[1], lead.cap);
        std::vector<uint32_t> us(cand_groups.size(), 0), ue(cand_groups.size(), 0);
        const int rc = [&] {
            if (!lead_ready || (!built && !search_leaders())) return (int)MG_OK;
            if (lead.tot[0] == 0 || lead.overflowed()) return (int)MG_OK;
            return sort_universes(us, ue) && choose_groups(us, ue) ? encode_groups() : (int)MG_OK;
        }();
        if (rc != MG_OK) return rc;
        if (sp->dgroups_host.empty()) { (void)hipGetLastError(); drop_dense(); }
        sp->build_ms += std::chrono::duration<double, std::milli>(std::chrono::steady_clock::now() - t_dense).count();
        if (ctx_opt(ctx, "MASHGPU_SPARSE_DBG")) {
            uint64_t rows_in = 0;
            for (auto &G : sp->dgroups_host) rows_in += G.g1 - G.g0;
            fprintf(stderr, "compare dense: %zu chains of related rows, %zu groups kept (%llu rows, widest universe %u words)\n", cand_groups.size(),
                    sp->dgroups_host.size(), (unsigned long long)rows_in, sp->dn_wmax);
        }
    }
    if (ctx_opt(ctx, "MASHGPU_SPARSE_DBG")) {
        fprintf(stderr, "compare sparse: index of %llu rows (%llu copies of earlier rows), s %u: %u entries, %u distinct, shared %llu, largest run %u, %.2f ms\n",
                (unsigned long long)n, (unsigned long long)sp->copies, s, E, sp->G, (unsigned long long)sp->shared, sp->max_group, sp->build_ms);
        fprintf(stderr, "compare sparse: rows %s; the copy gate had %u suspects\n",
                !sp->inv ? "in the table's order" : sp->phashes ? "in clustered order, copied" : "in clustered order, read in place", gate_suspects);
    }
    return MG_OK;
}

int SparseIndexBuild::run()
{
    int rc = MG_OK;
    if ((rc = scan_rows()) != MG_OK || stop) return rc;
    if ((rc = order_rows()) != MG_OK || stop) return rc;
    if ((rc = find_copies()) != MG_OK || stop) return rc;
    if ((rc = lay_out()) != MG_OK || stop) return rc;
    if ((rc = build_by_tiles()) != MG_OK || stop) return rc;
    if ((rc = build_by_sort()) != MG_OK || stop) return rc;
    if ((rc = check_build()) != MG_OK || stop) return rc;
    return dense_groups();
}

}

int table_sparse_index(mg_ctx *ctx, const mg_table *t, uint32_t s, bool clustered, mg_table::Sparse **out, uint32_t split)
{
    if (!clustered) split = 0;
    for (mg_table::Sparse *sp : t->sparse)
        if (sp->s == s && sp->clustered == clustered && sp->split == split) { *out = sp; return MG_OK; }
    mg_table::Sparse *sp = new mg_table::Sparse;
    sp->s = s;
    sp->clustered = clustered;
    sp->split = split;
    t->sparse.push_back(sp);
    *out = sp;
    auto unusable = [&](const char *why) { sp->usable = false; sp->why = why; return MG_OK; };
    const uint64_t n = t->n;
    if (n == 0) return unusable("empty table");
    if (n >= (1ull << 31)) return unusable("too many rows");
    sp->rs = mg::sparse_img_stride(s);
    if (n * sp->rs >= (1ull << 32)) return unusable("image index beyond 32 bits");
    HIP_TRY(ctx, hipSetDevice(ctx->device));
    SparseIndexBuild build(ctx, t, s, clustered, sp, split);
    prof_begin(ctx, ctx->prof_index);
    struct ProfEnd { mg_ctx *c; ~ProfEnd() { prof_end(c, c->prof_index); } } prof_end_guard{ctx};
    return build.run();
}
```

mash_amd/csrc/host_internal.h:

```cpp
#pragma once
#include <hip/hip_runtime.h>
#include <rccl/rccl.h>

#include <algorithm>
#include <chrono>
#include <cmath>
#include <condition_variable>
#include <memory>
#include <iterator>
#include <functional>
#include <map>
#include <mutex>
#include <queue>
#include <cstdio>
#include <cstdlib>
#include <cstring>
#include <string>
#include <system_error>
#include <thread>
#include <type_traits>
#include <vector>

#include "../../include/mashgpu.h"
#include "cluster_internal.h"
// ... 13 lines not shown
    double discover_per_shared = 2.0e-12;
    double discover_per_entry = 4.0e-11;
    double merge_per_candidate = 1.0e-9;
    double launches = 2.0e-5;
    double class_bytes_s = 2.0e12;
    double dense_per_pair = 3.0e-11;
    double tiles_rate_small = 8.0e9, tiles_rate_mid = 1.5e10, tiles_rate_large = 3.0e10;
    double tiles_per_shared = 8.0e-12;
    double join_per_shared = 2.2e-13;
    double join_per_step = 4.0e-11;
    double join_per_slot = 8.0e-11;
    double join_min_shared_per_pair = 4.0;
};


struct mg_ctx {
    int device = 0;
    hipStream_t stream = nullptr;
    bool own_stream = false;
    int cu_count = 0;
    std::string err;
    bool prof = false;
    std::vector<ProfRec> prof_compare, prof_sketch;
    std::vector<ProfRec> prof_fill, prof_discover, prof_merge, prof_index, prof_dense, prof_join;
    std::vector<ProfRec> prof_fill_aside;
    void *pin = nullptr;
    size_t pin_cap = 0;
    std::recursive_mutex mu;
    bool async = false;
    struct TileSlot { void *dev = nullptr, *host = nullptr; size_t cap = 0; hipEvent_t done = nullptr; bool pending = false; };
    TileSlot slots[4];
    unsigned slot_next = 0;
    struct Block { void *p; size_t bytes; };
    std::vector<Block> blk_free, blk_live;
    size_t blk_cached = 0;
    std::vector<Block> big_free;
    size_t big_cached = 0, big_limit = (size_t)48 << 30;
    std::map<std::string, std::string> options;
    uint64_t greedy_rounds = 0, greedy_batches = 0, greedy_regrows = 0, greedy_edge_cap = 0;
    uint64_t forest_rounds = 0, forest_regrows = 0, forest_edge_cap = 0;
    std::vector<uint64_t> forest_live, forest_chosen;
    SparseCosts costs;
    struct CostClock { hipEvent_t a = nullptr, b = nullptr; };
    CostClock cost_clk[5];
    uint64_t cost_updates = 0;
    hipStream_t aux = nullptr;
    hipEvent_t aux_go = nullptr, aux_done = nullptr;
    uint32_t *aux_ctr = nullptr;
    std::function<void(uint32_t)> aside_all_copies;
    std::function<void()> aside_at_sort;
};

struct mg_table {
    mg_ctx *ctx = nullptr;
    const uint64_t *hashes = nullptr;
    const uint32_t *nhash = nullptr;
    const uint64_t *lengths = nullptr;
    bool has_lengths = true;
    uint64_t n = 0, s = 0;
    bool owns = false;
    mutable bool have_max = false;
    mutable uint64_t maxval = 0;
    mutable std::vector<std::pair<int, uint32_t *>> pfx;
    mutable std::vector<uint8_t> cls;
    mutable std::vector<uint64_t> last;
    mutable std::vector<uint32_t> nh;
    struct Windows { int shr; uint32_t delta, nwin, s; uint32_t *dev; std::vector<uint32_t> host; };
    mutable std::vector<Windows> win;
    struct Sparse {
        uint32_t s = 0;
        bool usable = false;
        std::string why;
        uint32_t E = 0, G = 0, rs = 0;
        uint64_t shared = 0;
        uint32_t max_group = 0;
        double build_ms = 0;
        uint32_t *off = nullptr;
        std::vector<uint32_t> off_host;
        uint64_t *keys_sorted = nullptr;
        uint32_t *gend = nullptr;
        uint32_t *sorted_rows = nullptr;
        uint32_t *code_img = nullptr;
        uint32_t *pos_img = nullptr;
        uint32_t *order = nullptr;
        std::vector<mg::DenseGroup> dgroups_host;
        mg::DenseGroup *dgroups = nullptr;
        std::vector<uint32_t> grp_of_host;
        uint32_t *grp_of = nullptr;
        uint32_t *ulist = nullptr, *upos = nullptr;
        unsigned long long *gdata = nullptr;
        uint16_t *ext = nullptr;
        uint32_t dn_wmax = 0, dn_xs = 0;
        bool dn_lists = false;
        bool clustered = false;
        uint32_t split = 0;
        bool by_tiles = false;
        uint32_t *inv = nullptr;
        uint64_t *phashes = nullptr;
        uint32_t *rep = nullptr, *cls_of = nullptr, *cls_off = nullptr, *cls_rows = nullptr, *cls_first = nullptr;
        uint32_t cls_members = 0;
        uint64_t cls_pairs = 0;
        uint64_t copies = 0;
        uint64_t runs_dropped = 0;
        uint32_t one_class = 0;
        bool has_empty = false;
        uint32_t *short_rows = nullptr, *short_cnt = nullptr;
        std::vector<uint32_t> short_rows_host;
        struct Join {
            bool built = false, only_shared = false;
            bool ordered = false;
            uint32_t split = 0;
            mg::JoinSide side;
            const uint32_t *src = nullptr, *map = nullptr;
            void *bufs[9] = {nullptr, nullptr, nullptr, nullptr, nullptr, nullptr, nullptr, nullptr, nullptr};
            double build_ms = 0;
        } jn;
        struct Plan { const void *rows; uint64_t rb, re; bool triangle; uint64_t cand, shared; bool use; bool use_list; bool join; uint32_t *order;
                      mg::DenseTile *dtiles; uint32_t ndtiles, dtile_rows; uint64_t dense_pairs; };
        std::vector<Plan> plans;
        uint2 *cand = nullptr, *res = nullptr;
        uint64_t cand_cap = 0;
        unsigned long long *counters = nullptr;
        unsigned long long *seg_base = nullptr;
        uint32_t *seg_cnt = nullptr, *chunks = nullptr, *chunk_inc = nullptr;
        void *scan_temp = nullptr;
        size_t scan_temp_bytes = 0;
        uint64_t seg_rows = 0;
    };
    mutable std::vector<Sparse *> sparse;
    mutable std::vector<mg_table *> prefix_views;
};

#define HIP_TRY(ctx, call)                                                           \
    do {                                                                             \
        hipError_t e__ = (call);                                                     \
        if (e__ != hipSuccess) {                                                     \
            (ctx)->err = std::string(#call) + ": " + hipGetErrorString(e__);        \
            return MG_ERR_HIP;                                                       \
        }                                                                            \
    } while (0)


bool ctx_is_live(const void *c);
void ctx_trim(mg_ctx *ctx);
hipError_t ctx_malloc(mg_ctx *ctx, void **out, size_t bytes);
const mg_table *table_prefix_view(const mg_table *t, uint64_t n);
void ctx_free(mg_ctx *ctx, void *p);

template <class T>
struct DevBuf {
    T *p = nullptr;
    mg_ctx *owner = nullptr;
    DevBuf() = default;
    explicit DevBuf(mg_ctx *ctx) : owner(ctx) {}
    DevBuf(const DevBuf &) = delete;
    DevBuf &operator=(const DevBuf &) = delete;
    ~DevBuf() { free(); }
    void free() { if (p) { if (owner) ctx_free(owner, p); else hipFree(p); p = nullptr; } }
    hipError_t alloc(uint64_t count)
    {
        free();
        const size_t bytes = std::max<uint64_t>(count, 1) * sizeof(T);
        return owner ? ctx_malloc(owner, reinterpret_cast<void **>(&p), bytes) : hipMalloc(&p, bytes);
    }
    T *release() { T *q = p; p = nullptr; return q; }
    operator T *() const { return p; }
// ... 102 lines not shown
```

mash_amd/csrc/index_build.h:

```cpp
#pragma once
#include <stdint.h>

namespace mg {

struct IxGeom {
    uint32_t n, nblk, E;
    uint32_t shift;
    uint32_t bw_log, BW;
    uint32_t NW, Bp;
    uint32_t rb;
    uint32_t npass;
    uint32_t wgrp;
    uint32_t nseq;
    uint32_t rs;
    uint32_t want_gs;
    uint64_t stride;
};

struct IxLeaders {
    const uint32_t *grp_of = nullptr;
    unsigned long long *key = nullptr;
    uint32_t *val = nullptr;
    uint32_t *cnt = nullptr;
    uint32_t cap_sub = 0, nsub = 0;
};

struct IxPlan {
    IxGeom g;
    bool ok = false;
    const char *why = "";
    size_t lb_bytes = 0, cnt_bytes = 0, start_bytes = 0, big_bytes = 0, pk_bytes = 0, tc_bytes = 0;
};

enum { IXF_NSTREAMED = 0, IXF_DEGENERATE = 1, IXF_MAXBUCKET = 2, IXF_NBIG = 3 };

IxPlan index_plan(uint32_t n, uint32_t E, uint32_t s, uint32_t rs, uint64_t stride, uint64_t maxv, double dens0, bool want_gs);
size_t index_stat_scratch_bytes();
hipError_t index_debug_swap(const IxPlan &plan, void *pk, const void *start, uint32_t *done, hipStream_t stream);
hipError_t index_build(const IxPlan &plan, const uint64_t *hashes, const uint32_t *off, void *lb, void *cnt, void *start, void *big, void *pk, void *tc,
                       uint64_t *keys_sorted, uint32_t *sorted_rows, uint32_t *gend, uint32_t *gs_of, uint32_t *code_img, uint32_t *pos_img,
                       void *stat_scratch, unsigned long long *incidences, uint32_t *max_group, uint32_t *groups, uint32_t *flags,
                       const IxLeaders *leaders, hipStream_t stream, int stages = 7);
hipError_t index_build_mapped(const IxPlan &plan, const uint64_t *hashes, const uint32_t *rowmap, const uint32_t *off, void *lb, void *cnt, void *start,
                              void *big, void *pk, void *tc, uint64_t *keys_sorted, uint32_t *sorted_rows, uint32_t *gend, uint32_t *gs_of,
                              uint32_t *code_img, uint32_t *pos_img, void *stat_scratch, unsigned long long *incidences, uint32_t *max_group,
                              uint32_t *groups, uint32_t *flags, const IxLeaders *leaders, hipStream_t stream, int stages = 7);
hipError_t index_window_offsets(const IxPlan &plan, const uint64_t *hashes, const uint32_t *rowmap, const uint32_t *cnt_table, void *lb, hipStream_t stream);
bool index_offsets_counts_fits(const IxGeom &g);
hipError_t index_offsets_counts(const IxPlan &plan, const uint64_t *hashes, const uint32_t *rowmap, const uint32_t *cnt_table, void *lb, void *cnt,
                                uint32_t *flags, hipStream_t stream);
hipError_t index_gather_rows(const IxPlan &plan, const uint64_t *hashes, const uint32_t *inv, const uint32_t *cnt_table, uint64_t *out, void *lb,
                             hipStream_t stream);

hipError_t index_verify_words(const uint32_t *a, const uint32_t *b, const uint32_t *cond, uint32_t mode, uint64_t count, unsigned long long *out2,
                              hipStream_t stream);

}
```

mash_amd/csrc/index_build.hip:

```cpp
#ifdef MG_HIP_EMU
#include "hipemu.h"
#else
#include <hip/hip_runtime.h>
#define MG_DYN_SHARED(T, name)                                   \
    extern __shared__ __align__(16) unsigned char name##_raw[]; \
    T *name = reinterpret_cast<T *>(name##_raw)
#endif
#include <stdint.h>

#include <cstdio>
#include <cstdlib>
#include <cstring>

#include "index_build.h"

#ifdef MG_HIP_EMU
#define IX_IN_LANE_ORDER(stmt)                                   \
    for (uint32_t l_ = 0; l_ < 64u; l_++) {                     \
        if ((threadIdx.x & 63u) == l_) { stmt; }                \
        hipemu::wave_sync();                                     \
    }
#else
#define IX_IN_LANE_ORDER(stmt) { stmt; }
#endif
// ... 445 lines not shown
                atomicAdd(&s_hist[bl], 1u);
                s_pack[at[it]] = ((v[it] & lowmask) << g.rb) | (uint64_t)(row0 + r);
                s_pa[at[it]] = (bl << 12) | at[it];
            }
        }
#pragma unroll 1
        for (uint32_t r = tid / IX_LPR; r < nrows; r += IX_NT / IX_LPR) {
            const uint32_t rp = s_rowpre[r], ln = s_rowpre[r + 1u] - rp;
            if (ln <= IX_LPR || rp + ln <= i0 || rp >= i0 + np) continue;
            const uint64_t *src = H + (uint64_t)s_trow[r] * g.stride + s_lo[r];
            for (uint32_t k = sub + IX_LPR; k < ln; k += IX_LPR) {
                const uint32_t i = rp + k;
                if (i < i0 || i >= i0 + np) continue;
                const uint64_t x = src[k];
                const uint32_t bl = (uint32_t)(x >> g.shift) & (g.BW - 1u);
                atomicAdd(&s_hist[bl], 1u);
                s_pack[i - i0] = ((x & lowmask) << g.rb) | (uint64_t)(row0 + r);
                s_pa[i - i0] = (bl << 12) | (i - i0);
            }
        }
        __syncthreads();
        IX_CLK(1);
        uint32_t *srt = ix_tile_sort(s_pa, s_pb, s_cnt, s_part, np, g.npass);
        IX_CLK(2);
        uint32_t *s_slot = srt == s_pa ? s_pb : s_pa;
        {
            const uint32_t c = tid < g.BW ? s_hist[tid] : 0u;
            uint32_t tot = 0;
            const uint32_t ex = ix_block_scan_sum(c, s_part, tot);
            if (tid < g.BW) s_hist[tid] = ex;
            if (tid == 0) s_hist[g.BW] = np;
        }
        __syncthreads();
        IX_CLK(3);
        for (uint32_t j = tid; j < np; j += IX_NT) {
            const uint32_t e = srt[j], b = e >> 12, idx = e & 4095u;
            const uint32_t slot = s_gbase[b] + (j - s_hist[b]);
            pk[slot] = s_pack[idx];
            s_slot[idx] = slot;
        }
        __syncthreads();
        IX_CLK(4);
        {
            uint32_t sl[IX_ROUNDS], lo8[IX_ROUNDS];
#pragma unroll
            for (uint32_t it = 0; it < IX_ROUNDS; it++) {
                const uint32_t r = it * (IX_NT / IX_LPR) + tid / IX_LPR;
                sl[it] = s_slot[at[it] != 0xFFFFFFFFu ? at[it] : 0u];
                lo8[it] = s_lo[r < nrows ? r : 0u];
            }
#pragma unroll
            for (uint32_t it = 0; it < IX_ROUNDS; it++) {
                const uint32_t r = it * (IX_NT / IX_LPR) + tid / IX_LPR;
                if (at[it] != 0xFFFFFFFFu) slot_img[(uint64_t)(row0 + r) * g.rs + lo8[it] + sub] = sl[it];
            }
        }
#pragma unroll 1
        for (uint32_t r = tid / IX_LPR; r < nrows; r += IX_NT / IX_LPR) {
            const uint32_t rp = s_rowpre[r], ln = s_rowpre[r + 1u] - rp;
            if (ln <= IX_LPR || rp + ln <= i0 || rp >= i0 + np) continue;
            const uint64_t at0 = (uint64_t)(row0 + r) * g.rs + s_lo[r];
            for (uint32_t k = sub + IX_LPR; k < ln; k += IX_LPR) {
                const uint32_t i = rp + k;
                if (i >= i0 && i < i0 + np) slot_img[at0 + k] = s_slot[i - i0];
            }
        }
        IX_CLK(5);
        uint32_t add = 0;
        if (tid < g.BW) add = s_hist[tid + 1] - s_hist[tid];
        __syncthreads();
        if (tid < g.BW) {
            s_gbase[tid] += add;
            s_hist[tid] = 0;
        }
        s_trow[tid] = trow;
        __syncthreads();
    }
}

constexpr uint32_t IX5_CH = 32;
constexpr uint32_t IX5_UNR = 4;

__global__ __launch_bounds__(256) void ix_images_kernel(IxGeom g, const uint32_t *__restrict__ off, const uint32_t *__restrict__ flags,
                                                        const uint2 *__restrict__ tc, uint32_t *__restrict__ code_img, uint32_t *pos_img, uint32_t nchunk)
{
    const uint32_t per = gridDim.x >> 3;
    const uint32_t q = (blockIdx.x & 7u) * per + (blockIdx.x >> 3);
    if (q >= g.nblk * nchunk) return;
    const uint32_t blk = q / nchunk, ch = q - blk * nchunk;
    const uint32_t tid = threadIdx.x, quad = tid & 7u, rsub = tid >> 3;
    const uint32_t p0 = ch * IX5_CH + quad * 4u;
    const uint32_t row0 = blk * IX_RB, nrows = g.n - row0 < IX_RB ? g.n - row0 : IX_RB;
    uint32_t cnt_n[IX5_UNR];
    uint32_t sl_n[IX5_UNR][4];
    auto slots = [&](uint32_t rb) {
#pragma unroll
        for (uint32_t u = 0; u < IX5_UNR; u++) {
            const uint32_t r = rb + 32u * u;
            const uint32_t row = row0 + (r < nrows ? r : 0u);
            const uint32_t c = r < nrows ? off[row + 1u] - off[row] : 0u;
            cnt_n[u] = c;
            const uint32_t *src = pos_img + (uint64_t)row * g.rs + (p0 < c ? p0 : 0u);
            sl_n[u][0] = src[0];
            sl_n[u][1] = src[1];
            sl_n[u][2] = src[2];
            sl_n[u][3] = src[3];
        }
    };
    if (rsub < nrows) slots(rsub);
    for (uint32_t rb = rsub; rb < nrows; rb += 32u * IX5_UNR) {
        uint32_t cnt[IX5_UNR];
        uint32_t sl[IX5_UNR][4];
#pragma unroll
        for (uint32_t u = 0; u < IX5_UNR; u++) {
            cnt[u] = cnt_n[u];
#pragma unroll
            for (uint32_t e = 0; e < 4u; e++) sl[u][e] = sl_n[u][e];
        }
        uint2 cp[IX5_UNR][4];
#pragma unroll
        for (uint32_t u = 0; u < IX5_UNR; u++)
#pragma unroll
            for (uint32_t e = 0; e < 4u; e++) cp[u][e] = tc[p0 + e < cnt[u] ? sl[u][e] : 0u];
        if (rb + 32u * IX5_UNR < nrows) slots(rb + 32u * IX5_UNR);
#pragma unroll
        for (uint32_t u = 0; u < IX5_UNR; u++) {
            const uint32_t r = rb + 32u * u;
            if (r < nrows && p0 < g.rs) {
                const uint64_t at = (uint64_t)(row0 + r) * g.rs + p0;
#pragma unroll
                for (uint32_t e = 0; e < 4u; e++) {
                    code_img[at + e] = p0 + e < cnt[u] ? cp[u][e].x : 0xFFFFFFFFu;
                    if (p0 + e < cnt[u]) pos_img[at + e] = cp[u][e].y;
                }
            }
        }
    }
}

__device__ __forceinline__ uint32_t ix_subshift(const IxGeom &g) { return g.shift >= IX_SUBBITS ? g.shift + g.rb - IX_SUBBITS : g.rb; }

constexpr uint32_t IX4_PK = 0, IX4_JX = IX4_PK + IX_CAP * 8u, IX4_H = IX4_JX + IX_CAP * 2u, IX4_MIX = IX4_H + IX_NSUB * 2u,
                   IX4_PART = IX4_MIX + IX_NSUB / 8u, IX4_BYTES = IX4_PART + 64u;

template <bool PART> struct IxBodyPtr { using In = const uint64_t *__restrict__; using Keys = uint64_t *__restrict__; using Rows = uint32_t *__restrict__; };
template <> struct IxBodyPtr<true> { using In = const uint64_t *; using Keys = uint64_t *; using Rows = uint32_t *; };

template <uint32_t PER, bool PART>
__device__ __forceinline__ bool ix_bucket_sort_body(const IxGeom &g, typename IxBodyPtr<PART>::In src, const uint32_t *arr, uint32_t tcbase, uint32_t subshift,
                                                    typename IxBodyPtr<PART>::Keys keys_sorted, typename IxBodyPtr<PART>::Rows sorted_rows, uint32_t *__restrict__ gend,
                                                    uint32_t *__restrict__ gs_of, uint2 *__restrict__ tc, IxStatSlot *stat, uint32_t *flags,
                                                    const IxLeaders &lead, uint64_t *s_pk, uint16_t *s_jx, uint32_t *s_h, uint32_t *s_mixed,
                                                    uint32_t *s_part, uint32_t b, uint32_t G0, uint32_t N)
{
    const uint32_t tid = threadIdx.x, lane = tid & 63u, wave = tid >> 6;
    IX_CLK_BEGIN();
    for (uint32_t x = tid; x < IX_NSUB / 2u; x += IX_NT4) s_h[x] = 0;
    if (tid < IX_NSUB / 32u) s_mixed[tid] = 0;
    uint64_t v[PER];
    uint32_t sa[PER];
    uint32_t am[PART ? PER : 1u];
#pragma unroll
    for (uint32_t k = 0; k < PER; k++) {
        const uint32_t j = tid + k * IX_NT4;
        const bool in = j < N;
        const uint64_t x = src[in ? j : 0u];
        v[k] = x;
        if constexpr (PART) am[k] = arr[in ? j : 0u];
        const uint32_t sub0 = (uint32_t)(x >> subshift) & (IX_NSUB - 1u);
        if (in) s_jx[j] = (uint16_t)(((sub0 >> IX_SUBLOW) << 13) | (sub0 & ((1u << IX_SUBLOW) - 1u)));
    }
    __syncthreads();
    IX_CLK(32);
    uint16_t *s_tk = s_jx;
    for (uint32_t j0 = 0; j0 < N; j0 += 256u) {
        uint32_t tag[4];
#pragma unroll
        for (uint32_t u = 0; u < 4u; u++) {
            const uint32_t j = j0 + 64u * u + lane;
            tag[u] = j < N ? (uint32_t)s_tk[j] : 0xFFFFu;
        }
        uint32_t old[4];
#pragma unroll
        for (uint32_t u = 0; u < 4u; u++) {
            const uint32_t j = j0 + 64u * u + lane;
            const bool mine = (tag[u] >> 13) == wave && j < N;
            const uint32_t sub = (wave << IX_SUBLOW) | (tag[u] & ((1u << IX_SUBLOW) - 1u));
            const uint32_t h16 = (sub & 1u) * 16u;
            uint32_t o = 0;
            IX_IN_LANE_ORDER(if (mine) o = atomicAdd(&s_h[sub >> 1], 1u << h16));
            old[u] = (o >> h16) & 0xFFFFu;
        }
#pragma unroll
        for (uint32_t u = 0; u < 4u; u++) {
            const uint32_t j = j0 + 64u * u + lane;
            if ((tag[u] >> 13) == wave && j < N) s_tk[j] = (uint16_t)((wave << 13) | old[u]);
        }
    }
    __syncthreads();
    IX_CLK(33);
    {
        uint32_t wv[8], sum = 0;
#pragma unroll
        for (uint32_t x = 0; x < 8u; x++) {
            wv[x] = s_h[8u * tid + x];
            sum += (wv[x] & 0xFFFFu) + (wv[x] >> 16);
        }
        uint32_t total = 0;
        uint32_t run = ix_block_scan_sum(sum, s_part, total);
#pragma unroll
        for (uint32_t x = 0; x < 8u; x++) {
            const uint32_t lo = wv[x] & 0xFFFFu, hi = wv[x] >> 16;
            s_h[8u * tid + x] = run | ((run + lo) << 16);
            run += lo + hi;
        }
    }
    const uint16_t *cs = reinterpret_cast<const uint16_t *>(s_h);
// ... 423 lines not shown
                if constexpr (LEVEL == 1) {
                    ix_big_split(src_w + a, src_arr + a, alt_w + a, alt_arr + a, m, sshift_next, cs_next, lds, s_part);
                    ok = ix_big_walk<2>(g, alt_w + a, alt_arr + a, nullptr, nullptr, gpos + a, m, sshift_next, cs_next, nullptr, o, lead, lds, b, tcbase);
                }
            } else {
                if (threadIdx.x == 0) o.flags[IXF_DEGENERATE] = 1u;
                ok = false;
            }
            sub++;
        } else {
            const uint32_t cnt = ix_big_first(cs, lo) - a;
            if (cnt)
                ok = ix_bucket_sort_body<IX_CAP / IX_NT4, true>(g, src_w + a, src_arr + a, tcbase, lo == sub + 1u ? sshift_next : sshift, o.keys_sorted,
                                                                o.sorted_rows, o.gend, o.gs_of, o.tc, o.stat, o.flags, lead, s_pk, s_jx, s_h, s_mixed, s_part,
                                                                b, gpos + a, cnt);
            sub = lo;
        }
        if (!ok) return false;
        __syncthreads();
    }
    return true;
}

__global__ __launch_bounds__(IX_NT4, 2) void ix_big_bucket_kernel(IxGeom g, uint64_t *pk, const uint32_t *start, const uint32_t *biglist,
                                                               uint64_t *keys_sorted, uint32_t *sorted_rows, uint32_t *gend, uint32_t *gs_of, uint2 *tc,
                                                               IxStatSlot *stat, uint32_t *flags, IxLeaders lead)
{
    MG_DYN_SHARED(unsigned char, lds);
    uint32_t *s_part = reinterpret_cast<uint32_t *>(lds + IX4_PART);
    uint32_t *cs1 = reinterpret_cast<uint32_t *>(lds + IXB_CS1), *cs2 = reinterpret_cast<uint32_t *>(lds + IXB_CS2);
    const IxOut o{keys_sorted, sorted_rows, gend, gs_of, tc, stat, flags};
    const uint32_t nbig = flags[IXF_NBIG];
    const uint32_t sshift = ix_subshift(g);
    for (uint32_t i = blockIdx.x; i < nbig; i += gridDim.x) {
        const uint32_t b = biglist[i];
        const uint32_t G0 = start[b], N = start[b + 1] - G0;
        ix_big_split(pk + G0, nullptr, keys_sorted + G0, sorted_rows + G0, N, sshift, cs1, lds, s_part);
        if (!ix_big_walk<1>(g, keys_sorted + G0, sorted_rows + G0, pk + G0, gend + G0, G0, N, sshift, cs1, cs2, o, lead, lds, b, G0)) return;
        __syncthreads();
    }
}

__global__ __launch_bounds__(256) void ix_stat_reduce_kernel(const IxStatSlot *stat, unsigned long long *incidences, uint32_t *max_group, uint32_t *groups)
{
    unsigned long long inc = 0;
    uint32_t m = 0, gr = 0;
    for (uint32_t i = threadIdx.x; i < IX_STAT_SLOTS; i += 256u) {
        inc += stat[i].inc;
        m = stat[i].max_group > m ? stat[i].max_group : m;
        gr += stat[i].groups;
    }
    if (inc) atomicAdd(incidences, inc);
    if (m) atomicMax(max_group, m);
    if (gr) atomicAdd(groups, gr);
}

__global__ __launch_bounds__(256) void ix_fill_u32_kernel(uint32_t *p, uint64_t count, uint32_t v)
{
    const uint64_t stride = (uint64_t)gridDim.x * 256u;
    for (uint64_t i = (uint64_t)blockIdx.x * 256u + threadIdx.x; i < count; i += stride) p[i] = v;
}

__global__ __launch_bounds__(256) void ix_verify_kernel(const uint32_t *a, const uint32_t *b, const uint32_t *cond, uint32_t mode, uint64_t count,
                                                        unsigned long long *out)
{
    const uint64_t stride = (uint64_t)gridDim.x * 256u;
    for (uint64_t i = (uint64_t)blockIdx.x * 256u + threadIdx.x; i < count; i += stride) {
        if (mode == 1u && cond[i] != (uint32_t)i) continue;
        if (mode == 2u && cond[i] == 0xFFFFFFFFu) continue;
        if (a[i] != b[i]) {
            atomicAdd(&out[0], 1ull);
            atomicMin(&out[1], (unsigned long long)i);
        }
    }
}

hipError_t index_verify_words(const uint32_t *a, const uint32_t *b, const uint32_t *cond, uint32_t mode, uint64_t count, unsigned long long *out2,
                              hipStream_t stream)
{
    if (count == 0) return hipSuccess;
    uint64_t blocks = (count + 1023u) / 1024u;
    if (blocks > 8192u) blocks = 8192u;
    hipLaunchKernelGGL(ix_verify_kernel, dim3((uint32_t)blocks), dim3(256), 0, stream, a, b, cond, mode, count, out2);
    return hipGetLastError();
}


size_t index_stat_scratch_bytes() { return sizeof(IxStatSlot) * IX_STAT_SLOTS; }

#if defined(IX_PHASE_CLOCKS) && !defined(MG_HIP_EMU)
void index_dump_clocks()
{
    unsigned long long h[64];
    if (hipMemcpyFromSymbol(h, HIP_SYMBOL(ix_clk), sizeof h) != hipSuccess) return;
    static const char *k3[] = {"prologue (lb, scan, gbase)", "loads + pack", "tile sort", "bucket scan", "pk + slots to LDS", "slot image"};
    static const char *k4[] = {"zero + load", "tickets", "counter scan + ticket read", "scatter", "mixed mark + fix-up + write back", "heads + inverse", "out by position + leaders", "statistics + leaders' scan", "tc by arrival", "leaders out"};
    unsigned long long t3 = 0, t4 = 0;
    for (int i = 0; i < 6; i++) t3 += h[i];
    for (int i = 0; i < 10; i++) t4 += h[32 + i];
    for (int i = 0; i < 6; i++) fprintf(stderr, "ix clocks K3 %-34s %6.2f %%\n", k3[i], 100.0 * h[i] / (t3 ? t3 : 1));
    for (int i = 0; i < 10; i++) fprintf(stderr, "ix clocks K4 %-34s %6.2f %%\n", k4[i], 100.0 * h[32 + i] / (t4 ? t4 : 1));
    memset(h, 0, sizeof h);
    (void)hipMemcpyToSymbol(HIP_SYMBOL(ix_clk), h, sizeof h);
}
#endif

IxPlan index_plan(uint32_t n, uint32_t E, uint32_t s, uint32_t rs, uint64_t stride, uint64_t maxv, double dens0, bool want_gs)
{
    IxPlan p;
    IxGeom &g = p.g;
    g = IxGeom{};
    if (n == 0 || E == 0) { p.why = "empty"; return p; }
    if (s > 65535u) { p.why = "sketch size beyond 16-bit positions"; return p; }
    g.n = n;
    g.E = E;
    g.rs = rs;
    g.stride = stride;
    g.want_gs = want_gs ? 1u : 0u;
    g.nblk = (n + IX_RB - 1u) / IX_RB;
    g.rb = 1;
    while (g.rb < 32u && (1ull << g.rb) < (uint64_t)n) g.rb++;
    if (!(dens0 > 0.0)) { p.why = "no density"; return p; }
    uint32_t shift = 0;
    while (shift < 63u && dens0 * (double)(1ull << (shift + 1u)) <= IX_TMAX) shift++;
    if (shift > 64u - g.rb) shift = 64u - g.rb;
    if (shift > 63u) shift = 63u;
    g.shift = shift;
    const uint64_t B = (maxv >> shift) + 1ull;
    if (B > (1ull << 22)) { p.why = "too many buckets (values far from evenly spread)"; return p; }
    uint32_t bw_log = 0;
    while (bw_log < 9u && (1ull << (bw_log + 1u)) <= IX_BW_MAX && shift + bw_log + 1u <= 63u && (1ull << bw_log) < B &&
           (double)E * (double)(2u << bw_log) / ((double)g.nblk * (double)B) <= IX_TILE_TARGET)
        bw_log++;
    g.bw_log = bw_log;
    g.BW = 1u << bw_log;
    g.NW = (uint32_t)((B + g.BW - 1u) / g.BW);
    g.Bp = g.NW * g.BW;
    g.npass = (bw_log + 3u) / 4u;
    g.wgrp = 8;
    const uint64_t nseq = (uint64_t)((g.NW + g.wgrp - 1u) / g.wgrp) * g.wgrp * g.nblk;
    if (nseq >= (1ull << 30)) { p.why = "too many tiles"; return p; }
    g.nseq = (uint32_t)nseq;
    p.lb_bytes = (size_t)n * (g.NW + 1u) * 2u;
    p.cnt_bytes = (size_t)g.nblk * g.Bp * 4u;
    p.start_bytes = ((size_t)g.Bp + 1u) * 4u;
    p.pk_bytes = (size_t)E * 8u;
    p.tc_bytes = (size_t)E * 8u;
    p.big_bytes = ((size_t)E / IX_CAP + 2u) * 4u;
    if (p.lb_bytes > ((size_t)2 << 30) || p.cnt_bytes > ((size_t)2 << 30)) { p.why = "scratch of the tiles too large"; return p; }
    p.ok = true;
    return p;
}

hipError_t index_gather_rows(const IxPlan &plan, const uint64_t *hashes, const uint32_t *inv, const uint32_t *cnt_table, uint64_t *out, void *lb_v,
                             hipStream_t stream)
{
    if (!plan.ok) return hipErrorInvalidValue;
    hipLaunchKernelGGL(ix_gather_offsets_kernel, dim3(plan.g.n), dim3(256), 0, stream, plan.g, hashes, inv, cnt_table, out, static_cast<uint16_t *>(lb_v));
    return hipGetLastError();
}

__global__ __launch_bounds__(64) void ix_debug_swap_kernel(IxGeom g, uint64_t *pk, const uint32_t *start, uint32_t *done)
{
    if (threadIdx.x != 0) return;
    for (uint32_t b = 0; b < g.Bp; b++) {
        const uint32_t a = start[b], e = start[b + 1];
        if (e - a < 2u || e - a > IX_CAP) continue;
        for (uint32_t j = a; j + 1u < e; j++) {
            if ((pk[j] >> g.rb) == (pk[j + 1] >> g.rb)) {
                const uint64_t t = pk[j];
                pk[j] = pk[j + 1];
                pk[j + 1] = t;
                done[0] = 1u;
                return;
            }
        }
    }
}

hipError_t index_debug_swap(const IxPlan &plan, void *pk_v, const void *start_v, uint32_t *done, hipStream_t stream)
{
    if (!plan.ok) return hipErrorInvalidValue;
    hipLaunchKernelGGL(ix_debug_swap_kernel, dim3(1), dim3(64), 0, stream, plan.g, static_cast<uint64_t *>(pk_v), static_cast<const uint32_t *>(start_v), done);
    return hipGetLastError();
}

hipError_t index_window_offsets(const IxPlan &plan, const uint64_t *hashes, const uint32_t *rowmap, const uint32_t *cnt_table, void *lb_v, hipStream_t stream)
{
    if (!plan.ok) return hipErrorInvalidValue;
    hipLaunchKernelGGL(ix_window_offsets_kernel, dim3((plan.g.n + 3u) / 4u), dim3(256), 0, stream, plan.g, hashes, rowmap, (const uint32_t *)nullptr, cnt_table,
                       static_cast<uint16_t *>(lb_v));
    return hipGetLastError();
}

bool index_offsets_counts_fits(const IxGeom &g) { return ixoc_lds_bytes(g.Bp) <= IXOC_LDS_MAX; }

hipError_t index_offsets_counts(const IxPlan &plan, const uint64_t *hashes, const uint32_t *rowmap, const uint32_t *cnt_table, void *lb_v, void *cnt_v,
                                uint32_t *flags, hipStream_t stream)
{
    if (!plan.ok || !index_offsets_counts_fits(plan.g)) return hipErrorInvalidValue;
    const uint32_t lds = (uint32_t)ixoc_lds_bytes(plan.g.Bp);
    const hipError_t e = hipFuncSetAttribute(reinterpret_cast<const void *>(ix_offsets_counts_kernel), hipFuncAttributeMaxDynamicSharedMemorySize, (int)lds);
    if (e != hipSuccess) return e;
    hipLaunchKernelGGL(ix_offsets_counts_kernel, dim3(plan.g.nblk), dim3(IXOC_NT), lds, stream, plan.g, hashes, rowmap, cnt_table, static_cast<uint16_t *>(lb_v),
                       static_cast<uint32_t *>(cnt_v), flags);
    return hipGetLastError();
}

hipError_t index_build(const IxPlan &plan, const uint64_t *hashes, const uint32_t *off, void *lb_v, void *cnt_v, void *start_v, void *big_v, void *pk_v, void *tc_v,
                       uint64_t *keys_sorted, uint32_t *sorted_rows, uint32_t *gend, uint32_t *gs_of, uint32_t *code_img, uint32_t *pos_img,
                       void *stat_scratch, unsigned long long *incidences, uint32_t *max_group, uint32_t *groups, uint32_t *flags,
                       const IxLeaders *leaders, hipStream_t stream, int stages)
{
    return index_build_mapped(plan, hashes, nullptr, off, lb_v, cnt_v, start_v, big_v, pk_v, tc_v, keys_sorted, sorted_rows, gend, gs_of, code_img, pos_img,
                              stat_scratch, incidences, max_group, groups, flags, leaders, stream, stages);
}

hipError_t index_build_mapped(const IxPlan &plan, const uint64_t *hashes, const uint32_t *rowmap, const uint32_t *off, void *lb_v, void *cnt_v, void *start_v,
                              void *big_v, void *pk_v, void *tc_v, uint64_t *keys_sorted, uint32_t *sorted_rows, uint32_t *gend, uint32_t *gs_of,
                              uint32_t *code_img, uint32_t *pos_img, void *stat_scratch, unsigned long long *incidences, uint32_t *max_group,
                              uint32_t *groups, uint32_t *flags, const IxLeaders *leaders, hipStream_t stream, int stages)
{
    if (!plan.ok) return hipErrorInvalidValue;
    const IxGeom g = plan.g;
    uint16_t *lb = static_cast<uint16_t *>(lb_v);
    uint32_t *cnt = static_cast<uint32_t *>(cnt_v), *start = static_cast<uint32_t *>(start_v);
    uint64_t *pk = static_cast<uint64_t *>(pk_v);
    uint2 *tc = static_cast<uint2 *>(tc_v);
    hipError_t e = hipSuccess;
    if (stages & 1) {
        e = hipFuncSetAttribute(reinterpret_cast<const void *>(ix_tile_partition_kernel), hipFuncAttributeMaxDynamicSharedMemorySize, (int)IXL_BYTES);
        if (e != hipSuccess) return e;
        const uint32_t tiles = 8u * ((g.nseq + 7u) / 8u);
        if (!(stages & (8 | 16))) hipLaunchKernelGGL(ix_window_offsets_kernel, dim3((g.n + 3u) / 4u), dim3(256), 0, stream, g, hashes, rowmap, off,
                                                     (const uint32_t *)nullptr, lb);
        if (!(stages & 16)) hipLaunchKernelGGL(ix_tile_count_kernel, dim3(tiles), dim3(IX_NT), 0, stream, g, hashes, rowmap, (const uint16_t *)lb, cnt);
        hipLaunchKernelGGL(ix_col_scan_kernel, dim3((g.Bp + 255u) / 256u), dim3(256), 0, stream, g, cnt, start);
        hipLaunchKernelGGL(ix_bucket_scan_kernel, dim3(1), dim3(1024), 0, stream, g, start, flags, static_cast<uint32_t *>(big_v));
        e = hipGetLastError();
        if (e != hipSuccess) return e;
        hipLaunchKernelGGL(ix_tile_partition_kernel, dim3(tiles), dim3(IX_NT), IXL_BYTES, stream, g, hashes, rowmap, (const uint16_t *)lb, (const uint32_t *)cnt,
                           (const uint32_t *)start, (const uint32_t *)flags, pk, pos_img);
        e = hipGetLastError();
        if (e != hipSuccess) return e;
    }
    if (stages & 2) {
        e = hipFuncSetAttribute(reinterpret_cast<const void *>(ix_bucket_sort_kernel), hipFuncAttributeMaxDynamicSharedMemorySize, (int)IX4_BYTES);
        if (e == hipSuccess) e = hipFuncSetAttribute(reinterpret_cast<const void *>(ix_big_bucket_kernel), hipFuncAttributeMaxDynamicSharedMemorySize, (int)IXB_BYTES);
        if (e != hipSuccess) return e;
        e = hipMemsetAsync(stat_scratch, 0, index_stat_scratch_bytes(), stream);
        if (e != hipSuccess) return e;
        hipLaunchKernelGGL(ix_bucket_sort_kernel, dim3(g.Bp), dim3(IX_NT4), IX4_BYTES, stream, g, (const uint64_t *)pk, (const uint32_t *)start, keys_sorted,
                           sorted_rows, gend, g.want_gs ? gs_of : (uint32_t *)nullptr, tc, static_cast<IxStatSlot *>(stat_scratch), flags,
                           leaders ? *leaders : IxLeaders());
        hipLaunchKernelGGL(ix_big_bucket_kernel, dim3(256), dim3(IX_NT4), IXB_BYTES, stream, g, pk, (const uint32_t *)start,
                           (const uint32_t *)big_v, keys_sorted, sorted_rows, gend, g.want_gs ? gs_of : (uint32_t *)nullptr, tc,
                           static_cast<IxStatSlot *>(stat_scratch), flags, leaders ? *leaders : IxLeaders());
        hipLaunchKernelGGL(ix_stat_reduce_kernel, dim3(1), dim3(256), 0, stream, static_cast<const IxStatSlot *>(stat_scratch), incidences, max_group, groups);
    }
    if (!(stages & 4)) return hipGetLastError();
    {
        const uint32_t nchunk = (g.rs + IX5_CH - 1u) / IX5_CH;
        const uint32_t pieces = 8u * ((g.nblk * nchunk + 7u) / 8u);
        hipLaunchKernelGGL(ix_images_kernel, dim3(pieces), dim3(256), 0, stream, g, off, (const uint32_t *)flags, (const uint2 *)tc, code_img, pos_img, nchunk);
    }
    return hipGetLastError();
}

}
```

mash_amd/csrc/mashgpu.cpp:

```cpp
#include "host_internal.h"

namespace {

thread_local std::string g_create_error;

std::mutex g_live_mu;
std::vector<const void *> g_live_ctx;

}

bool ctx_is_live(const void *c)
{
    std::lock_guard<std::mutex> lk(g_live_mu);
    return std::find(g_live_ctx.begin(), g_live_ctx.end(), c) != g_live_ctx.end();
}

void ctx_trim(mg_ctx *ctx)
{
    for (auto &b : ctx->blk_free) hipFree(b.p);
    ctx->blk_free.clear();
    ctx->blk_cached = 0;
    for (auto &b : ctx->big_free) hipFree(b.p);
    ctx->big_free.clear();
    ctx->big_cached = 0;
// ... 222 lines not shown
    HIP_TRY(ctx, hipSetDevice(ctx->device));
    HIP_TRY(ctx, hipStreamSynchronize(ctx->stream));
    return MG_OK;
}

int mg_ctx_cu_count(mg_ctx *ctx) { return ctx ? ctx->cu_count : 0; }

int mg_params_init(mg_params *p, int kmer_size, uint64_t sketch_size, uint32_t seed,
                   const char *alphabet, int noncanonical, int preserve_case)
{
    if (!p || !alphabet || kmer_size < 1 || kmer_size > 32 || sketch_size < 1) return MG_ERR_INVALID;
    memset(p, 0, sizeof *p);
    p->kmer_size = kmer_size;
    p->sketch_size = sketch_size;
    p->seed = seed;
    p->noncanonical = noncanonical ? 1 : 0;
    p->preserve_case = preserve_case ? 1 : 0;
    p->min_copies = 1;
    p->target_cov = 0.0;
    p->bloom_bytes = 0;
    for (const char *c = alphabet; *c; c++) {
        char u = *c;
        if (!preserve_case && u > 96 && u < 123) u -= 32;
        p->alphabet[(unsigned char)u] = 1;
    }
    for (int i = 0; i < 256; i++) p->alphabet_size += p->alphabet[i] ? 1 : 0;
    p->use64 = pow((double)p->alphabet_size, (double)kmer_size) > pow(2.0, 32.0);
    return MG_OK;
}


int mg_table_upload(mg_ctx *ctx, const uint64_t *hashes, const uint32_t *nhash, const uint64_t *lengths,
                    uint64_t n, uint64_t s, mg_table **out)
{
    if (!ctx) return MG_ERR_INVALID;
    std::lock_guard<std::recursive_mutex> lk(ctx->mu);
    if (!hashes || !nhash || !out || s == 0) return fail(ctx, MG_ERR_INVALID, "mg_table_upload: bad argument");
    HIP_TRY(ctx, hipSetDevice(ctx->device));
    DevBuf<uint64_t> dh(ctx), dl(ctx);
    DevBuf<uint32_t> dn(ctx);
    if (dh.alloc(n * s) != hipSuccess || dn.alloc(n) != hipSuccess || dl.alloc(n) != hipSuccess)
        return fail(ctx, MG_ERR_NOMEM, "mg_table_upload: device allocation failed");
    HIP_TRY(ctx, hipMemcpyAsync(dh, hashes, n * s * 8, hipMemcpyHostToDevice, ctx->stream));
    HIP_TRY(ctx, hipMemcpyAsync(dn, nhash, n * 4, hipMemcpyHostToDevice, ctx->stream));
    if (lengths) HIP_TRY(ctx, hipMemcpyAsync(dl, lengths, n * 8, hipMemcpyHostToDevice, ctx->stream));
    else HIP_TRY(ctx, hipMemsetAsync(dl, 0, n * 8, ctx->stream));
    HIP_TRY(ctx, hipStreamSynchronize(ctx->stream));
    mg_table *t = new mg_table;
    t->ctx = ctx; t->hashes = dh.release(); t->nhash = dn.release(); t->lengths = dl.release(); t->n = n; t->s = s; t->owns = true;
    t->has_lengths = lengths != nullptr;
    *out = t;
    return MG_OK;
}

int mg_table_wrap_dev(mg_ctx *ctx, const uint64_t *hashes_dev, const uint32_t *nhash_dev,
                      const uint64_t *lengths_dev, uint64_t n, uint64_t s, mg_table **out)
{
    if (!ctx) return MG_ERR_INVALID;
    std::lock_guard<std::recursive_mutex> lk(ctx->mu);
    if (!hashes_dev || !nhash_dev || !out || s == 0) return fail(ctx, MG_ERR_INVALID, "mg_table_wrap_dev: bad argument");
    mg_table *t = new mg_table;
    t->ctx = ctx; t->hashes = hashes_dev; t->nhash = nhash_dev; t->lengths = lengths_dev;
    t->n = n; t->s = s; t->owns = false;
    *out = t;
    return MG_OK;
}

static void table_drop_derived(mg_table *t)
{
    mg_ctx *ctx = t->ctx;
    for (mg_table *v : t->prefix_views) { table_drop_derived(v); delete v; }
    t->prefix_views.clear();
    if (!t->pfx.empty() || !t->win.empty() || !t->sparse.empty()) hipSetDevice(ctx->device);
    for (auto &im : t->pfx) ctx_free(ctx, im.second);
    t->pfx.clear();
    for (auto &w : t->win) ctx_free(ctx, w.dev);
    t->win.clear();
    for (mg_table::Sparse *sp : t->sparse) {
        for (auto &pl : sp->plans) {
            if (pl.order) ctx_free(ctx, pl.order);
            if (pl.dtiles) ctx_free(ctx, pl.dtiles);
        }
        for (void *q : {(void *)sp->off, (void *)sp->keys_sorted, (void *)sp->gend, (void *)sp->sorted_rows,
                        (void *)sp->pos_img, (void *)sp->code_img, (void *)sp->short_rows, (void *)sp->short_cnt, (void *)sp->cand,
                        (void *)sp->res, (void *)sp->seg_base, (void *)sp->seg_cnt, (void *)sp->chunks, (void *)sp->chunk_inc,
                        sp->scan_temp, (void *)sp->counters, (void *)sp->rep, (void *)sp->cls_of, (void *)sp->cls_off,
                        (void *)sp->cls_rows, (void *)sp->cls_first, (void *)sp->order, (void *)sp->dgroups, (void *)sp->grp_of,
                        (void *)sp->ulist, (void *)sp->upos, (void *)sp->gdata, (void *)sp->ext, (void *)sp->inv, (void *)sp->phashes})
            if (q) ctx_free(ctx, q);
        for (void *q : sp->jn.bufs)
            if (q) ctx_free(ctx, q);
        delete sp;
    }
    t->sparse.clear();
    t->cls.clear();
    t->last.clear();
    t->nh.clear();
    t->have_max = false;
}

const mg_table *table_prefix_view(const mg_table *t, uint64_t n)
{
    if (n >= t->n) return t;
    for (mg_table *v : t->prefix_views)
        if (v->n == n) return v;
    if (t->prefix_views.size() >= 4) {
        table_drop_derived(t->prefix_views.front());
        delete t->prefix_views.front();
        t->prefix_views.erase(t->prefix_views.begin());
    }
    mg_table *v = new mg_table;
    v->ctx = t->ctx;
    v->hashes = t->hashes;
    v->nhash = t->nhash;
    v->lengths = t->lengths;
    v->has_lengths = t->has_lengths;
    v->n = n;
    v->s = t->s;
    v->owns = false;
    t->prefix_views.push_back(v);
    return v;
}

void mg_table_free(mg_table *t)
{
    if (!t) return;
    if (!ctx_is_live(t->ctx)) { delete t; return; }
    {
        std::lock_guard<std::recursive_mutex> lk(t->ctx->mu);
        table_drop_derived(t);
        if (t->owns) {
            hipSetDevice(t->ctx->device);
            ctx_free(t->ctx, (void *)t->hashes);
            ctx_free(t->ctx, (void *)t->nhash);
            ctx_free(t->ctx, (void *)t->lengths);
        }
    }
    delete t;
}

int mg_table_invalidate(mg_table *t)
{
    if (!t || !ctx_is_live(t->ctx)) return MG_ERR_INVALID;
    std::lock_guard<std::recursive_mutex> lk(t->ctx->mu);
    table_drop_derived(t);
    return MG_OK;
}

uint64_t mg_table_rows(const mg_table *t) { return t ? t->n : 0; }
uint64_t mg_table_sketch_size(const mg_table *t) { return t ? t->s : 0; }


int mg_prof_enable(mg_ctx *ctx, int on)
{
    if (!ctx) return MG_ERR_INVALID;
    std::lock_guard<std::recursive_mutex> lk(ctx->mu);
    ctx->prof = on != 0;
    return MG_OK;
}

void mg_prof_reset(mg_ctx *ctx)
{
    if (!ctx) return;
    for (auto *v : {&ctx->prof_compare, &ctx->prof_sketch, &ctx->prof_fill, &ctx->prof_discover, &ctx->prof_merge, &ctx->prof_index, &ctx->prof_dense, &ctx->prof_join, &ctx->prof_fill_aside}) {
        for (auto &r : *v) { hipEventDestroy(r.a); hipEventDestroy(r.b); }
        v->clear();
    }
// ... 29 lines not shown
```

Baseline: 441.0 billion pairs/s.

## Compute per-row partner flags during index build to skip rows in discover

The image-building and dense-encode kernels now record, for each row, whether any of its hashes maps to a group whose end differs from its start, meaning the row has partners. The discover kernel reads this flag and returns early for rows without partners, instead of rescanning each row's code and position segments. This adds a memset, some ballots and atomics in the index build, plus an optional verify kernel. It also changes the loop bounds in the images kernel so whole 8-row groups take part in the ballot.

```diff
diff --git a/mash_amd/csrc/compare_dense.hip b/mash_amd/csrc/compare_dense.hip
--- a/mash_amd/csrc/compare_dense.hip
+++ b/mash_amd/csrc/compare_dense.hip
@@ -185,11 +185,20 @@
 
 constexpr uint32_t DN_CX_MASK = 0x7FFFu, DN_CX_FLAG = 0x8000u;
 
+struct DnEncodeOpts {
+    uint32_t ul_in_lds;
+    uint32_t *row_any;
+#ifdef __HIPCC__
+    __host__ __device__
+#endif
+    DnEncodeOpts(uint32_t ul, uint32_t *flags = nullptr) : ul_in_lds(ul), row_any(flags) {}
+};
+
 template <uint32_t DN_EK>
 __global__ __launch_bounds__(256) void dn_encode_kernel(const uint32_t *off, const uint32_t *code_img, uint32_t *pos_img, uint32_t rs,
                                                         const uint32_t *grp_of, const DenseGroup *groups, const uint32_t *ulist,
                                                         const uint32_t *upos, unsigned long long *gdata, uint32_t wstride, uint16_t *ext,
-                                                        uint32_t xs, uint32_t n, uint32_t ul_in_lds)
+                                                        uint32_t xs, uint32_t n, DnEncodeOpts opt)
 {
     MG_DYN_SHARED(uint32_t, lds);
     const uint32_t bid = blockIdx.x;
@@ -204,13 +213,15 @@
     uint32_t *ull = lds + 28u * wstride + 9u;
     for (uint32_t i = tid; i < 28u * W + 1u; i += 256u) lds[i] = 0;
     const uint32_t *ulg = ulist + G.ustart, *up = upos + G.ustart;
-    if (ul_in_lds)
+    if (opt.ul_in_lds)
         for (uint32_t i = tid; i < u; i += 256u) ull[i] = ulg[i];
-    const uint32_t *ul = ul_in_lds ? ull : ulg;
+    const uint32_t *ul = opt.ul_in_lds ? ull : ulg;
+    if (tid == 0) scr[4] = 0;
     __syncthreads();
     const uint32_t cnt = off[row + 1] - off[row];
     uint16_t *xrow = ext + (uint64_t)(G.xrow0 + (row - G.g0)) * xs;
     uint32_t nx = 0;
+    bool any = false;
     if constexpr (DN_EK == 1) {
         for (uint32_t base = 0; base < cnt; base += 256u) {
             const uint32_t p = base + tid;
@@ -218,7 +229,7 @@
             bool extra = false;
             if (p < cnt) {
                 const uint64_t img = (uint64_t)row * rs + p;
-                const uint32_t gs = code_img[img] >> 1;
+                const uint32_t code = code_img[img], gs = code >> 1;
                 uint32_t lo = 0, hi = u;
                 while (lo < hi) {
                     const uint32_t mid = (lo + hi) >> 1;
@@ -227,9 +238,12 @@
                 idx = lo;
                 if (lo < u && ul[lo] == gs) {
                     atomicOr(&mask32[idx >> 5], 1u << (idx & 31u));
-                    pos_img[img] = up[idx];
+                    const uint32_t end = up[idx];
+                    pos_img[img] = end;
+                    any |= end != gs;
                 } else {
                     extra = true;
+                    if (opt.row_any && (code & 1u)) any |= pos_img[img] != gs;
                 }
             }
             const uint64_t bal = __ballot(extra);
@@ -297,6 +311,7 @@
                                 if (j == nxt) xidx[j] = pos;
                             nxt++;
                         }
+                        any |= pv[e] != gs;
                     }
                 }
                 pp[0] = make_uint4(pv[0], pv[1], pv[2], pv[3]);
@@ -327,7 +342,9 @@
             __syncthreads();
         }
     }
+    if (__ballot(any) != 0 && lane == 0) atomicOr(&scr[4], 1u);
     __syncthreads();
+    if (opt.row_any && tid == 0) opt.row_any[row] = scr[4];
     const uint32_t jb = (row - G.g0) >> 7, bl = (row - G.g0) & 127u;
     const uint64_t bw = dense_block_words(W);
     unsigned long long *blk = gdata + G.data_off + (uint64_t)jb * bw;
@@ -367,7 +384,7 @@
 
 hipError_t launch_dense_encode(const uint32_t *off, const uint32_t *code_img, uint32_t *pos_img, uint32_t rs, const uint32_t *grp_of,
                                const DenseGroup *groups, const uint32_t *ulist, const uint32_t *upos, unsigned long long *gdata,
-                               uint16_t *ext, uint32_t xs, uint32_t n, uint32_t wmax, hipStream_t stream, int ul_mode)
+                               uint16_t *ext, uint32_t xs, uint32_t n, uint32_t wmax, hipStream_t stream, int ul_mode, uint32_t *row_any)
 {
     if (n == 0) return hipSuccess;
     const size_t fixed = ((size_t)28 * wmax + 9) * 4, with_ul = fixed + (size_t)wmax * 64 * 4;
@@ -377,7 +394,7 @@
         hipError_t e = hipFuncSetAttribute(reinterpret_cast<const void *>(kern), hipFuncAttributeMaxDynamicSharedMemorySize, (int)smem);
         if (e != hipSuccess) return e;
         hipLaunchKernelGGL(kern, dim3((n + 63u) & ~63u), dim3(256), smem, stream, off, code_img, pos_img, rs, grp_of, groups, ulist, upos, gdata, wmax, ext, xs,
-                           n, ul_in_lds ? 1u : 0u);
+                           n, DnEncodeOpts(ul_in_lds ? 1u : 0u, row_any));
         return hipGetLastError();
     };
     return rs >= 4096u ? go(dn_encode_kernel<8>) : go(dn_encode_kernel<1>);
diff --git a/mash_amd/csrc/compare_internal.h b/mash_amd/csrc/compare_internal.h
--- a/mash_amd/csrc/compare_internal.h
+++ b/mash_amd/csrc/compare_internal.h
@@ -68,6 +68,7 @@
     const uint32_t *lo_img;
     const uint32_t *hi_img;
     uint32_t lo_shift;
+    const uint32_t *row_any = nullptr;
     const uint32_t *off;
     const uint32_t *row_img;
     const uint32_t *col_img;
@@ -197,7 +198,8 @@
                                 uint32_t group_bits, hipStream_t stream);
 hipError_t launch_dense_encode(const uint32_t *off, const uint32_t *code_img, uint32_t *pos_img, uint32_t rs, const uint32_t *grp_of,
                                const DenseGroup *groups, const uint32_t *ulist, const uint32_t *upos, unsigned long long *gdata,
-                               uint16_t *ext, uint32_t xs, uint32_t n, uint32_t wmax, hipStream_t stream, int ul_mode = -1);
+                               uint16_t *ext, uint32_t xs, uint32_t n, uint32_t wmax, hipStream_t stream, int ul_mode = -1,
+                               uint32_t *row_any = nullptr);
 size_t dense_pairs_lds(uint32_t W, uint32_t rows);
 uint32_t dense_rows_per_tile(uint64_t wave_rows);
 uint32_t dense_max_words();
diff --git a/mash_amd/csrc/compare_sparse.hip b/mash_amd/csrc/compare_sparse.hip
--- a/mash_amd/csrc/compare_sparse.hip
+++ b/mash_amd/csrc/compare_sparse.hip
@@ -623,9 +623,10 @@
     const uint32_t W = (ncols + 31u) >> 5;
     const uint32_t er = (DEDUP && a.triangle) ? a.rep[row] : row;
     const bool copy = DEDUP && a.triangle && er != row;
+    if (!copy && a.row_any != nullptr && a.row_any[er] == 0u) return;
     const uint32_t cnt = a.off[er + 1] - a.off[er];
     if (cnt == 0 || ncols == 0) return;
-    if (!copy) {
+    if (!copy && a.row_any == nullptr) {
         int any = 0;
         for (uint32_t p = tid; p < cnt; p += 256u) {
             const uint64_t at = (uint64_t)er * a.rs_row + p;
diff --git a/mash_amd/csrc/host_compare.cpp b/mash_amd/csrc/host_compare.cpp
--- a/mash_amd/csrc/host_compare.cpp
+++ b/mash_amd/csrc/host_compare.cpp
@@ -613,6 +613,8 @@
         a.lo_img = ix->code_img;
         a.hi_img = ix->pos_img;
         a.lo_shift = 1;
+        const char *flags_opt = ctx_opt(ctx, "MASHGPU_DISCOVER_ROWFLAGS");
+        a.row_any = ix->by_tiles && !(flags_opt && atoi(flags_opt) == 0) ? ix->row_any : nullptr;
         a.off = ix->off;
         a.row_img = ix->code_img;
         a.rs_row = ix->rs;
@@ -658,6 +660,7 @@
         a.lo_img = q_lo;
         a.hi_img = q_hi;
         a.lo_shift = 0;
+        a.row_any = nullptr;
         a.off = q_off;
         a.row_img = q_img;
         a.rs_row = rsq;
@@ -786,6 +789,8 @@
     want = first ? std::max<uint64_t>(ix->cand_cap, std::min<uint64_t>(pairs, std::min<uint64_t>(std::max<uint64_t>((uint64_t)ix->E / 2, 1u << 16), 1ull << 27)))
                           : plan->cand;
     nothing_to_find = triangle && ix->one_class != 0;
+    if (!nothing_to_find && ctx_opt(ctx, "MASHGPU_SPARSE_DBG"))
+        fprintf(stderr, "compare discover: %s\n", a.row_any ? "rows without partners known by their flags" : "every row's segment scanned");
     for (int attempt = 0; !nothing_to_find; attempt++) {
         rc = ensure_lists(want);
         if (rc != MG_OK) return rc;
diff --git a/mash_amd/csrc/host_index.cpp b/mash_amd/csrc/host_index.cpp
--- a/mash_amd/csrc/host_index.cpp
+++ b/mash_amd/csrc/host_index.cpp
@@ -163,7 +163,7 @@
     void drop()
     {
             for (void **q : {(void **)&sp->off, (void **)&sp->keys_sorted, (void **)&sp->gend, (void **)&sp->sorted_rows, (void **)&sp->code_img,
-                             (void **)&sp->pos_img, (void **)&sp->short_rows, (void **)&sp->short_cnt, (void **)&sp->counters, (void **)&sp->order,
+                             (void **)&sp->pos_img, (void **)&sp->row_any, (void **)&sp->short_rows, (void **)&sp->short_cnt, (void **)&sp->counters, (void **)&sp->order,
                              (void **)&sp->rep, (void **)&sp->cls_of, (void **)&sp->cls_off, (void **)&sp->cls_rows, (void **)&sp->cls_first})
                 if (*q) { ctx_free(ctx, *q); *q = nullptr; }
     }
@@ -188,7 +188,7 @@
         const mg::IxLeaders lv = lead.view(d_lead_rows);
         return mg::index_build_mapped(plan, H, rowmap, sp->off, d_lb, d_tcnt, w.start, w.big, w.pk, w.tc, sp->keys_sorted, sp->sorted_rows, sp->gend, gs_of, sp->code_img,
                                sp->pos_img, d_slots, &d_stat.p->shared, &d_stat.p->max_group, &d_stat.p->groups, d_stat.p->ixf, lead_ready ? &lv : nullptr,
-                               ctx->stream, stages);
+                               ctx->stream, stages, sp->row_any);
     }
     hipError_t sort_buckets(const TileScratch &w)
     {
@@ -216,6 +216,7 @@
     bool choose_groups(const std::vector<uint32_t> &us, const std::vector<uint32_t> &ue);
     int encode_groups();
     int dense_groups();
+    int check_row_flags();
     int run();
 };
 
@@ -514,7 +515,7 @@
               d_slots.alloc(std::max(mg::sparse_stat_scratch_bytes(), mg::index_stat_scratch_bytes())) == hipSuccess &&
               (!want_order || (key64_a.alloc(n) == hipSuccess && key64_b.alloc(n) == hipSuccess));
     ok = ok && take(&sp->off, n + 1) && take(&sp->keys_sorted, E) && take(&sp->gend, E) && take(&sp->sorted_rows, E) &&
-         take(&sp->code_img, (size_t)n * sp->rs + 64) && take(&sp->pos_img, (size_t)n * sp->rs) && take(&sp->counters, 4) &&
+         take(&sp->code_img, (size_t)n * sp->rs + 64) && take(&sp->pos_img, (size_t)n * sp->rs) && take(&sp->row_any, n) && take(&sp->counters, 4) &&
          (!want_order || take(&sp->order, n));
     const size_t nshort = sp->short_rows_host.size();
     short_cnt.assign(nshort, 0);
@@ -777,7 +778,8 @@
     if (e == hipSuccess) e = hipMemcpyAsync(sp->grp_of, grp_of_h.data(), n * 4, hipMemcpyHostToDevice, ctx->stream);
     if (e == hipSuccess)
         e = mg::launch_dense_encode(sp->off, sp->code_img, sp->pos_img, sp->rs, sp->grp_of, sp->dgroups, sp->ulist, sp->upos, sp->gdata, sp->ext, sp->dn_xs,
-                                    (uint32_t)n, sp->dn_wmax, ctx->stream, ctx_opt(ctx, "MASHGPU_DENSE_UL_LDS") ? atoi(ctx_opt(ctx, "MASHGPU_DENSE_UL_LDS")) : -1);
+                                    (uint32_t)n, sp->dn_wmax, ctx->stream, ctx_opt(ctx, "MASHGPU_DENSE_UL_LDS") ? atoi(ctx_opt(ctx, "MASHGPU_DENSE_UL_LDS")) : -1,
+                                    sp->by_tiles ? sp->row_any : nullptr);
     sp->grp_of_host.swap(grp_of_h);
     if (e != hipSuccess) {
         drop();
@@ -820,6 +822,24 @@
     return MG_OK;
 }
 
+int SparseIndexBuild::check_row_flags()
+{
+    if (!ix_verify || !sp->by_tiles || !sp->usable) return MG_OK;
+    DevBuf<unsigned long long> d_diff(ctx);
+    if (d_diff.alloc(2) != hipSuccess) return no_memory();
+    unsigned long long diff[2] = {0, ~0ull};
+    hipError_t e = hipMemcpyAsync(d_diff, diff, sizeof diff, hipMemcpyHostToDevice, ctx->stream);
+    if (e == hipSuccess) e = mg::index_verify_row_flags(sp->off, sp->code_img, sp->pos_img, sp->rs, sp->row_any, (uint32_t)n, d_diff, ctx->stream);
+    if (e == hipSuccess) e = hipMemcpyAsync(diff, d_diff, sizeof diff, hipMemcpyDeviceToHost, ctx->stream);
+    if (e == hipSuccess) e = hipStreamSynchronize(ctx->stream);
+    if (e != hipSuccess) return lost(e);
+    if (diff[0]) {
+        sp->usable = false;
+        return fail(ctx, MG_ERR_INVALID, "index verify: row flags -- " + std::to_string(diff[0]) + " differ, first at row " + std::to_string(diff[1]));
+    }
+    return MG_OK;
+}
+
 int SparseIndexBuild::run()
 {
     int rc = MG_OK;
@@ -830,7 +850,8 @@
     if ((rc = build_by_tiles()) != MG_OK || stop) return rc;
     if ((rc = build_by_sort()) != MG_OK || stop) return rc;
     if ((rc = check_build()) != MG_OK || stop) return rc;
-    return dense_groups();
+    if ((rc = dense_groups()) != MG_OK || stop) return rc;
+    return check_row_flags();
 }
 
 }
diff --git a/mash_amd/csrc/host_internal.h b/mash_amd/csrc/host_internal.h
--- a/mash_amd/csrc/host_internal.h
+++ b/mash_amd/csrc/host_internal.h
@@ -119,6 +119,7 @@
         uint32_t *sorted_rows = nullptr;
         uint32_t *code_img = nullptr;
         uint32_t *pos_img = nullptr;
+        uint32_t *row_any = nullptr;
         uint32_t *order = nullptr;
         std::vector<mg::DenseGroup> dgroups_host;
         mg::DenseGroup *dgroups = nullptr;
diff --git a/mash_amd/csrc/index_build.h b/mash_amd/csrc/index_build.h
--- a/mash_amd/csrc/index_build.h
+++ b/mash_amd/csrc/index_build.h
@@ -40,11 +40,12 @@
 hipError_t index_build(const IxPlan &plan, const uint64_t *hashes, const uint32_t *off, void *lb, void *cnt, void *start, void *big, void *pk, void *tc,
                        uint64_t *keys_sorted, uint32_t *sorted_rows, uint32_t *gend, uint32_t *gs_of, uint32_t *code_img, uint32_t *pos_img,
                        void *stat_scratch, unsigned long long *incidences, uint32_t *max_group, uint32_t *groups, uint32_t *flags,
-                       const IxLeaders *leaders, hipStream_t stream, int stages = 7);
+                       const IxLeaders *leaders, hipStream_t stream, int stages = 7, uint32_t *row_any = nullptr);
 hipError_t index_build_mapped(const IxPlan &plan, const uint64_t *hashes, const uint32_t *rowmap, const uint32_t *off, void *lb, void *cnt, void *start,
                               void *big, void *pk, void *tc, uint64_t *keys_sorted, uint32_t *sorted_rows, uint32_t *gend, uint32_t *gs_of,
                               uint32_t *code_img, uint32_t *pos_img, void *stat_scratch, unsigned long long *incidences, uint32_t *max_group,
-                              uint32_t *groups, uint32_t *flags, const IxLeaders *leaders, hipStream_t stream, int stages = 7);
+                              uint32_t *groups, uint32_t *flags, const IxLeaders *leaders, hipStream_t stream, int stages = 7,
+                              uint32_t *row_any = nullptr);
 hipError_t index_window_offsets(const IxPlan &plan, const uint64_t *hashes, const uint32_t *rowmap, const uint32_t *cnt_table, void *lb, hipStream_t stream);
 bool index_offsets_counts_fits(const IxGeom &g);
 hipError_t index_offsets_counts(const IxPlan &plan, const uint64_t *hashes, const uint32_t *rowmap, const uint32_t *cnt_table, void *lb, void *cnt,
@@ -54,5 +55,7 @@
 
 hipError_t index_verify_words(const uint32_t *a, const uint32_t *b, const uint32_t *cond, uint32_t mode, uint64_t count, unsigned long long *out2,
                               hipStream_t stream);
+hipError_t index_verify_row_flags(const uint32_t *off, const uint32_t *code_img, const uint32_t *pos_img, uint32_t rs, const uint32_t *row_any, uint32_t n,
+                                  unsigned long long *out2, hipStream_t stream);
 
 }
diff --git a/mash_amd/csrc/index_build.hip b/mash_amd/csrc/index_build.hip
--- a/mash_amd/csrc/index_build.hip
+++ b/mash_amd/csrc/index_build.hip
@@ -551,7 +551,8 @@
 constexpr uint32_t IX5_UNR = 4;
 
 __global__ __launch_bounds__(256) void ix_images_kernel(IxGeom g, const uint32_t *__restrict__ off, const uint32_t *__restrict__ flags,
-                                                        const uint2 *__restrict__ tc, uint32_t *__restrict__ code_img, uint32_t *pos_img, uint32_t nchunk)
+                                                        const uint2 *__restrict__ tc, uint32_t *__restrict__ code_img, uint32_t *pos_img, uint32_t nchunk,
+                                                        uint32_t *__restrict__ row_any)
 {
     const uint32_t per = gridDim.x >> 3;
     const uint32_t q = (blockIdx.x & 7u) * per + (blockIdx.x >> 3);
@@ -576,8 +577,8 @@
             sl_n[u][3] = src[3];
         }
     };
-    if (rsub < nrows) slots(rsub);
-    for (uint32_t rb = rsub; rb < nrows; rb += 32u * IX5_UNR) {
+    if ((rsub & ~7u) < nrows) slots(rsub);
+    for (uint32_t rb = rsub; (rb & ~7u) < nrows; rb += 32u * IX5_UNR) {
         uint32_t cnt[IX5_UNR];
         uint32_t sl[IX5_UNR][4];
 #pragma unroll
@@ -591,17 +592,26 @@
         for (uint32_t u = 0; u < IX5_UNR; u++)
 #pragma unroll
             for (uint32_t e = 0; e < 4u; e++) cp[u][e] = tc[p0 + e < cnt[u] ? sl[u][e] : 0u];
-        if (rb + 32u * IX5_UNR < nrows) slots(rb + 32u * IX5_UNR);
+        if (((rb + 32u * IX5_UNR) & ~7u) < nrows) slots(rb + 32u * IX5_UNR);
 #pragma unroll
         for (uint32_t u = 0; u < IX5_UNR; u++) {
             const uint32_t r = rb + 32u * u;
+            bool any = false;
             if (r < nrows && p0 < g.rs) {
                 const uint64_t at = (uint64_t)(row0 + r) * g.rs + p0;
 #pragma unroll
                 for (uint32_t e = 0; e < 4u; e++) {
                     code_img[at + e] = p0 + e < cnt[u] ? cp[u][e].x : 0xFFFFFFFFu;
-                    if (p0 + e < cnt[u]) pos_img[at + e] = cp[u][e].y;
+                    if (p0 + e < cnt[u]) {
+                        pos_img[at + e] = cp[u][e].y;
+                        any |= (cp[u][e].x >> 1) != cp[u][e].y;
+                    }
                 }
+            }
+            if (row_any != nullptr) {
+                const uint64_t votes = __ballot(any);
+                const uint32_t half = (tid & 32u) ? (uint32_t)(votes >> 32) : (uint32_t)votes;
+                if (quad == 0 && ((half >> (tid & 24u)) & 0xFFu) != 0) atomicOr(&row_any[row0 + r], 1u);
             }
         }
     }
@@ -1191,6 +1201,32 @@
     uint64_t blocks = (count + 1023u) / 1024u;
     if (blocks > 8192u) blocks = 8192u;
     hipLaunchKernelGGL(ix_verify_kernel, dim3((uint32_t)blocks), dim3(256), 0, stream, a, b, cond, mode, count, out2);
+    return hipGetLastError();
+}
+
+__global__ __launch_bounds__(256) void ix_verify_row_flags_kernel(const uint32_t *off, const uint32_t *code_img, const uint32_t *pos_img, uint32_t rs,
+                                                                  const uint32_t *row_any, uint32_t n, unsigned long long *out)
+{
+    const uint32_t row = blockIdx.x * 4u + (threadIdx.x >> 6), lane = threadIdx.x & 63u;
+    if (row >= n) return;
+    const uint32_t cnt = off[row + 1u] - off[row];
+    bool any = false;
+    for (uint32_t p = lane; p < cnt; p += 64u) {
+        const uint64_t at = (uint64_t)row * rs + p;
+        any |= (code_img[at] >> 1) != pos_img[at];
+    }
+    const bool want = __ballot(any) != 0;
+    if (lane == 0 && want != (row_any[row] != 0u)) {
+        atomicAdd(&out[0], 1ull);
+        atomicMin(&out[1], (unsigned long long)row);
+    }
+}
+
+hipError_t index_verify_row_flags(const uint32_t *off, const uint32_t *code_img, const uint32_t *pos_img, uint32_t rs, const uint32_t *row_any, uint32_t n,
+                                  unsigned long long *out2, hipStream_t stream)
+{
+    if (n == 0) return hipSuccess;
+    hipLaunchKernelGGL(ix_verify_row_flags_kernel, dim3((n + 3u) / 4u), dim3(256), 0, stream, off, code_img, pos_img, rs, row_any, n, out2);
     return hipGetLastError();
 }
 
@@ -1319,16 +1355,16 @@
 hipError_t index_build(const IxPlan &plan, const uint64_t *hashes, const uint32_t *off, void *lb_v, void *cnt_v, void *start_v, void *big_v, void *pk_v, void *tc_v,
                        uint64_t *keys_sorted, uint32_t *sorted_rows, uint32_t *gend, uint32_t *gs_of, uint32_t *code_img, uint32_t *pos_img,
                        void *stat_scratch, unsigned long long *incidences, uint32_t *max_group, uint32_t *groups, uint32_t *flags,
-                       const IxLeaders *leaders, hipStream_t stream, int stages)
+                       const IxLeaders *leaders, hipStream_t stream, int stages, uint32_t *row_any)
 {
     return index_build_mapped(plan, hashes, nullptr, off, lb_v, cnt_v, start_v, big_v, pk_v, tc_v, keys_sorted, sorted_rows, gend, gs_of, code_img, pos_img,
-                              stat_scratch, incidences, max_group, groups, flags, leaders, stream, stages);
+                              stat_scratch, incidences, max_group, groups, flags, leaders, stream, stages, row_any);
 }
 
 hipError_t index_build_mapped(const IxPlan &plan, const uint64_t *hashes, const uint32_t *rowmap, const uint32_t *off, void *lb_v, void *cnt_v, void *start_v,
                               void *big_v, void *pk_v, void *tc_v, uint64_t *keys_sorted, uint32_t *sorted_rows, uint32_t *gend, uint32_t *gs_of,
                               uint32_t *code_img, uint32_t *pos_img, void *stat_scratch, unsigned long long *incidences, uint32_t *max_group,
-                              uint32_t *groups, uint32_t *flags, const IxLeaders *leaders, hipStream_t stream, int stages)
+                              uint32_t *groups, uint32_t *flags, const IxLeaders *leaders, hipStream_t stream, int stages, uint32_t *row_any)
 {
     if (!plan.ok) return hipErrorInvalidValue;
     const IxGeom g = plan.g;
@@ -1371,7 +1407,12 @@
     {
         const uint32_t nchunk = (g.rs + IX5_CH - 1u) / IX5_CH;
         const uint32_t pieces = 8u * ((g.nblk * nchunk + 7u) / 8u);
-        hipLaunchKernelGGL(ix_images_kernel, dim3(pieces), dim3(256), 0, stream, g, off, (const uint32_t *)flags, (const uint2 *)tc, code_img, pos_img, nchunk);
+        if (row_any != nullptr) {
+            e = hipMemsetAsync(row_any, 0, (size_t)g.n * 4u, stream);
+            if (e != hipSuccess) return e;
+        }
+        hipLaunchKernelGGL(ix_images_kernel, dim3(pieces), dim3(256), 0, stream, g, off, (const uint32_t *)flags, (const uint2 *)tc, code_img, pos_img, nchunk,
+                           row_any);
     }
     return hipGetLastError();
 }
diff --git a/mash_amd/csrc/mashgpu.cpp b/mash_amd/csrc/mashgpu.cpp
--- a/mash_amd/csrc/mashgpu.cpp
+++ b/mash_amd/csrc/mashgpu.cpp
@@ -328,7 +328,7 @@
             if (pl.dtiles) ctx_free(ctx, pl.dtiles);
         }
         for (void *q : {(void *)sp->off, (void *)sp->keys_sorted, (void *)sp->gend, (void *)sp->sorted_rows,
-                        (void *)sp->pos_img, (void *)sp->code_img, (void *)sp->short_rows, (void *)sp->short_cnt, (void *)sp->cand,
+                        (void *)sp->pos_img, (void *)sp->code_img, (void *)sp->row_any, (void *)sp->short_rows, (void *)sp->short_cnt, (void *)sp->cand,
                         (void *)sp->res, (void *)sp->seg_base, (void *)sp->seg_cnt, (void *)sp->chunks, (void *)sp->chunk_inc,
                         sp->scan_temp, (void *)sp->counters, (void *)sp->rep, (void *)sp->cls_of, (void *)sp->cls_off,
                         (void *)sp->cls_rows, (void *)sp->cls_first, (void *)sp->order, (void *)sp->dgroups, (void *)sp->grp_of,
```

Result: faster. 448.5 billion pairs/s (median of 6 runs) (+1.7%).
